# jfjlaros/HUMID

Hardware: AMD Instinct MI355X
Metric: reads/sec deduplicated, 10M PE150 UMI=8 d=1 (higher is better)
Workload: dtype u64; 1 GPU; 10000000 reads/GPU x 1 GPU (one shuffled read set of 10000000 reads, sliced by input order), PE150 UMI=8 in header -> 24-nt packed words (8+8+8), d=1, directional clustering; synthetic molecules=N/4, family 1+Geom(3), p_sub=1e-3, p_N=1e-4; reads_per_gpu=10000000, word_nt=24, distance=1, method=directional

## Files before the change

humid_amd/csrc/humid_exchange.hip:

```cpp
#include "pipeline.hip.h"

extern "C" {

static int compact_nodes_impl(humid_ctx *c, const uint64_t *d_edges, uint64_t n_edges, uint32_t record_stride, u64 id_bound,
                              const uint32_t **d_nodes, uint64_t *n_nodes, const uint64_t **d_compact_edges,
                              const uint32_t **d_node_counts);
static int combo_route_wide(humid_ctx *c, const W2 *d_word, const u32 *d_count, u32 n, u64 id_base, const ComboPlan &plan,
                            u32 combo, u32 n_ranks, const Item3 **d_items, u64 *counts);
static int pairs_keyed_wide(humid_ctx *c, const void *d_items, u32 n, bool interleaved, u64 id_base, const u32 *d_count,
                            const ComboPlan &plan, u32 combo, u32 distance, const u64 **d_records, u64 *n_edges);
static int stage_pairs_share(humid_ctx *c, const u64 *g_word, u32 U, u32 word_nt, u32 distance, u32 part_rank, u32 part_world,
                             u64 *n_edges_out);
namespace {
struct XRange { u64 lo = 1, hi = 0; };

void x_splitters(const std::vector<u64> &hist, u32 P, u32 word_nt, u32 bits, std::vector<XRange> &out) {
  const u32 shift = 2 * word_nt - bits;
  const size_t n_bins = hist.size();
  std::vector<u64> cum(n_bins);
  u64 total = 0;
  for (size_t i = 0; i < n_bins; i++) { total += hist[i]; cum[i] = total; }
  std::vector<size_t> bounds{0};
  for (u32 k = 1; k < P; k++) {
    const u64 target = (total * k + P - 1) / P;
// ... 254 lines not shown
    const void *gw = lw;
    const u32 *gc = lc;
    if (moves && u_total) {
      ENSURE(c->xo_gw, u_total * wb + 16);
      ENSURE(c->xo_gc, u_total * 4 + 16);
      ENSURE(c->s_word, 16);
      ENSURE(c->s_cnt, 16);
      TRY(x_exchange(c, cm, c->s_word.p, ucnt, true, c->xo_gw.p, ucnt, wb));
      TRY(x_exchange(c, cm, c->s_cnt.p, ucnt, true, c->xo_gc.p, ucnt, 4));
      gw = c->xo_gw.p;
      gc = c->xo_gc.as<u32>();
    }
    u64 e_raw = 0;
    if (u_total > 1) {
      if (wide) TRY(edit_edges<W2>(c, (const W2 *)gw, (u32)u_total, n, d, &e_raw, r, P, false));
      else TRY(edit_edges<u64>(c, (const u64 *)gw, (u32)u_total, n, d, &e_raw, r, P, false));
    }
    u64 raw_from[MAX_RANKS], raw_all = 0;
    TRY(x_host_gather(c, cm, &e_raw, 8, raw_from));
    for (u32 q = 0; q < P; q++) raw_all += raw_from[q];
    if (raw_all >= 0x7fffffffull) return fail(c, HUMID_E_OVERFLOW, "too many candidate pairs in the edit-distance search");
    const u64 *all_raw = c->e_raw.as<u64>();
    if (moves && raw_all) {
      ENSURE(c->xo_cross, raw_all * 8 + 16);
      ENSURE(c->e_raw, 16);
      u64 rs[MAX_RANKS];
      for (u32 q = 0; q < P; q++) rs[q] = e_raw;
      TRY(x_exchange(c, cm, c->e_raw.p, rs, true, c->xo_cross.p, raw_from, 8));
      all_raw = c->xo_cross.as<u64>();
    }
    u64 E_e = 0;
    if (raw_all) TRY(unique_edges(c, all_raw, raw_all, (u32)u_total, &E_e));
    XT("edit joins");
    const u32 n_ids = (u32)u_total;
    const u32 nw = (((n_ids + 31) / 32) + 7) & ~7u, nblk = nw / 8;
    c->cg_valid = false;
    c->cg_nblocks = nblk;
    ENSURE(c->cg_bits, (size_t)nw * 4);
    ENSURE(c->cg_nbits, (size_t)nw * 4);
    ENSURE(c->cg_cur, (size_t)(ER_REGIONS * ER_STRIDE + 8) * 4);
    ENSURE(c->xo_cnt, 64 * 4);
    {
      ZeroList z;
      memset(&z, 0, sizeof z);
      z.p[0] = c->cg_bits.as<u32>(); z.n[0] = nw;
      z.p[1] = c->cg_nbits.as<u32>(); z.n[1] = nw;
      z.p[2] = (u32 *)&c->d_ctr[CTR_EDGES]; z.n[2] = 2 * (CTR_GOVER - CTR_EDGES + 1);
      z.p[3] = c->cg_cur.as<u32>(); z.n[3] = ER_REGIONS * ER_STRIDE + 8;
      hipLaunchKernelGGL(k_zero_many, dim3(64), dim3(256), 0, st, z);
    }
    CgStatus cgs;
    u64 M_e = 0;
    if (E_e) {
      hipLaunchKernelGGL(k_mark_pairs, dim3(blocks_for(E_e)), dim3(256), 0, st, (const u64 *)c->e_edges.as<u64>(), (u32)E_e, n_ids,
                         c->cg_bits.as<u32>(), (u32 *)&c->d_ctr[CTR_OVERFULL]);
      CgSource src;
      src.er.e = nullptr; src.er.cap_r = 0; src.er.cur = c->cg_cur.as<u32>(); src.er.far = c->e_edges.as<u64>(); src.er.n_far = (u32)E_e;
      src.recs = nullptr; src.n_recs = 0; src.segs = nullptr; src.cnt_by_id = gc; src.n_ids = n_ids;
      src.pairs_bound = E_e;
      TRY(mark_stage(c, c->ev[EV_GRAPH_BUILT]));
      TRY(cg_build(c, src, method, cgs));
      if (c->h_ctr[CTR_OVERFULL]) return fail(c, HUMID_E_INVALID, "internal: an edit-distance pair outside the unique words");
      M_e = cgs.M;
      TRY(cg_cluster_rest(c, n_ids, cgs.M, cgs.Mbig, method));
    } else {
      ENSURE(c->cg_blk, ((size_t)nblk + 1) * 4);
      ENSURE(c->cg_nblk, ((size_t)nblk + 1) * 4);
      HIPCHK(hipMemsetAsync(c->cg_blk.p, 0, ((size_t)nblk + 1) * 4, st));
      HIPCHK(hipMemsetAsync(c->cg_nblk.p, 0, ((size_t)nblk + 1) * 4, st));
    }
    const GraphArrays cg = cg_arrays(c);
    const BitRank br_in{c->cg_bits.as<u32>(), c->cg_blk.as<u32>()}, br_nc{c->cg_nbits.as<u32>(), c->cg_nblk.as<u32>()};
    const u32 *l_cid = nullptr;
    const u8 *l_ismax = nullptr;
    if (u_local) {
      ENSURE(c->x_lcid, (size_t)u_local * 4);
      ENSURE(c->x_lismax, (size_t)u_local);
      ENSURE(c->xo_ldeg, (size_t)u_local * 4);
      hipLaunchKernelGGL(k_own_results, dim3(blocks_for(u_local)), dim3(256), 0, st, br_in, br_nc, br_nc, (const u32 *)nullptr,
                         (const u32 *)c->cg_nodes.as<u32>(), (const u32 *)cg.cl_of, (const u32 *)cg.maxleaf, (const u32 *)cg.deg, (u32)goff,
                         (u32)u_local, 0u, c->x_lcid.as<u32>(), c->x_lismax.as<u8>(), c->xo_ldeg.as<u32>(),
                         (const u32 *)c->s_first.as<u32>(), (const u32 *)c->s_slot.as<u32>(), c->slot_out.as<u64>(), true);
      c->slots_done = true;
      l_cid = c->x_lcid.as<u32>();
      l_ismax = c->x_lismax.as<u8>();
    }
    HIPCHK(hipGetLastError());
    TRY(read_counters(c, c->cg_nblk.as<u32>() + nblk));
    const u64 clusters_e = u_total - (c->h_ctr[CTR_N - 1] & 0xffffffffull);
    if (clusters_e >= (1ull << 31)) return fail(c, HUMID_E_OVERFLOW, "cluster ids exceed 31 bits");
    XT("graph+ids");
    const u32 *packed = nullptr;
    u64 n_packed = 0;
    TRY(humid_stage_map_dense(c, l_cid, l_ismax, &packed, &n_packed));
    if (n_packed != n_recv) return fail(c, HUMID_E_INVALID, "map_dense returned %llu reads, %llu were counted", (ull)n_packed, (ull)n_recv);
    const u32 *ret = packed;
    if (moves && usable_all) {
      ENSURE(c->xr_ret, n_send * 4 + 8);
      TRY(x_exchange(c, cm, packed, recv_counts, false, c->xr_ret.p, send_counts, 4));
      ret = c->xr_ret.as<u32>();
    }
    if (n_local)
      hipLaunchKernelGGL(k_gather_results, dim3(grid_stride_blocks(n_local)), dim3(256), 0, st, (const u32 *)c->xo_inv.as<u32>(), ret,
                         (u32)n_send, (u32)n_local, d_cluster_id, d_keep);
    HIPCHK(hipGetLastError());
    HIPCHK(hipStreamSynchronize(st));
    XT("return");
    if (xtrace) fprintf(stderr, "[xtrace] rank %u/%u (edit distance) |%s\n", r, P, xt_line.c_str());
    if (summary) {
      memset(summary, 0, sizeof *summary);
      summary->total = total;
      summary->usable = usable;
      summary->unique = u_total;
      summary->clusters = clusters_e;
      summary->edges = E_e;
      summary->nonsingle = M_e;
      summary->ms_total = std::chrono::duration<float, std::milli>(std::chrono::steady_clock::now() - t_begin).count();
    }
    if (info) {
      info->unique_local = u_local;
      info->id_base = goff;
      info->n_nodes = M_e;
      info->n_pairs = E_e;
      info->d_unique_count = lc;
      info->d_unique_degree = u_local ? c->xo_ldeg.as<u32>() : nullptr;
    }
    return HUMID_OK;
  }
  u64 e_mine = 0;
  auto append_pairs = [&](const u64 *rec, u64 n_rec) -> int {
    if (!n_rec) return HUMID_OK;
    HIPCHK(c->xr_eloc.grow_keeping(e_mine * 16, (e_mine + n_rec) * 16, st));
    HIPCHK(hipMemcpyAsync(c->xr_eloc.as<u8>() + e_mine * 16, rec, n_rec * 16, hipMemcpyDeviceToDevice, st));
    e_mine += n_rec;
    return HUMID_OK;
  };
  auto discover_dense = [&]() -> int {
    if (d > 0 && u_total > 1) {
      u32 n_combos = 0, pb2 = 0;
      TRY(humid_stage_plan_info(c, n, d, u_total, &n_combos, &pb2));
      const ComboPlan wplan = make_plan(n, d, u_total, c->force_segments);
      const u64 ibytes = wide ? sizeof(Item3) : 16;
      const u64 *rec = nullptr;
      u64 n_rec = 0;
      if (u_local > 1) {
        if (wide) TRY(pairs_keyed_wide(c, lw, (u32)u_local, false, goff, lc, wplan, 0, d, &rec, &n_rec));
        else TRY(humid_stage_pairs_keyed(c, lw, u_local, 0, goff, lc, n, d, u_total, 0, &rec, &n_rec));
        TRY(append_pairs(rec, n_rec));
      }
      for (u32 cb = 1; cb < n_combos; cb++) {
        const u64 *items = nullptr;
        u64 sc[MAX_RANKS] = {0}, all_sc[MAX_RANKS * MAX_RANKS], rc[MAX_RANKS];
        if (wide) {
          const Item3 *it3 = nullptr;
          TRY(combo_route_wide(c, (const W2 *)lw, lc, (u32)u_local, goff, wplan, cb, P, &it3, sc));
          items = (const u64 *)it3;
        } else
          TRY(humid_stage_combo_route(c, lw, lc, u_local, goff, n, d, u_total, cb, P, &items, sc));
        TRY(x_host_gather(c, cm, sc, P * 8, all_sc));
        u64 n_got = 0;
        for (u32 q = 0; q < P; q++) { rc[q] = all_sc[(size_t)q * P + r]; n_got += rc[q]; }
        if (n_got > 0x7fffffffull) return fail(c, HUMID_E_OVERFLOW, "%llu unique words arrive at rank %u for one combination", (ull)n_got, r);
        u64 items_all = 0;
        for (u32 q = 0; q < P * P; q++) items_all += all_sc[q];
        const u64 *got = items;
        if (moves && items_all) {
// ... 264 lines not shown
  memset(&gs, 0, sizeof gs);
  CgStatus cgs;
  u64 M_mine = 0;
  if (n_recs_all) {
    u32 n_max = 1;
    for (u32 q = 0; q < REC_SEGS; q++) n_max = std::max(n_max, segs.n[q]);
    hipLaunchKernelGGL(k_mark_segs, dim3(std::min<u32>(blocks_for(n_max), 4096), REC_SEGS), dim3(256), 0, st, segs, n_ids,
                       c->cg_bits.as<u32>(), x_bad);
    CgSource src;
    src.er.e = nullptr; src.er.cap_r = 0; src.er.cur = c->cg_cur.as<u32>(); src.er.far = nullptr; src.er.n_far = 0;
    src.recs = nullptr; src.n_recs = 0; src.segs = &segs; src.cnt_by_id = nullptr; src.n_ids = n_ids;
    src.pairs_bound = n_recs_all;
    TRY(mark_stage(c, c->ev[EV_GRAPH_BUILT]));
    TRY(cg_build(c, src, method, cgs));
    if (c->h_ctr[CTR_OVERFULL]) return fail(c, HUMID_E_INVALID, "a pair record with an index outside the unique words");
    M_mine = cgs.M;
    TRY(cg_cluster_rest(c, n_ids, cgs.M, cgs.Mbig, method));
  } else {
    ENSURE(c->cg_blk, ((size_t)nblk + 1) * 4);
    ENSURE(c->cg_nblk, ((size_t)nblk + 1) * 4);
    HIPCHK(hipMemsetAsync(c->cg_blk.p, 0, ((size_t)nblk + 1) * 4, st));
    HIPCHK(hipMemsetAsync(c->cg_nblk.p, 0, ((size_t)nblk + 1) * 4, st));
  }
  const GraphArrays cg = cg_arrays(c);
  const BitRank br_in{c->cg_bits.as<u32>(), c->cg_blk.as<u32>()}, br_nc{c->cg_nbits.as<u32>(), c->cg_nblk.as<u32>()};
  BitRank br_xc{c->xo_xcbits.as<u32>(), c->xo_xcblk.as<u32>()};

  XT("graph");
  u64 C_x = 0;
  if (X_total && M_mine) {
    ENSURE(c->xo_xroot, (size_t)M_mine + 16);
    HIPCHK(hipMemsetAsync(c->xo_xroot.p, 0, (size_t)M_mine, st));
    hipLaunchKernelGGL(k_flag_xroots, dim3(std::min<u32>(blocks_for(X_total), 4096)), dim3(256), 0, st, segs, 1u, n_ids, br_in,
                       (const u32 *)cg.parent, c->xo_xroot.as<u8>(), by_count);
    hipLaunchKernelGGL(k_xcreator_bits, dim3(blocks_for(M_mine)), dim3(256), 0, st, (const u32 *)cg.cl_of, (const u32 *)cg.parent,
                       (const u8 *)c->xo_xroot.as<u8>(), (const u32 *)c->cg_nodes.as<u32>(), (u32)M_mine, c->xo_xcbits.as<u32>());
  }
  if (X_total) {
    TRY(exscan_in<u32>(c, BitsBlockIn{c->xo_xcbits.as<u32>(), nblk}, c->xo_xcblk.as<u32>(), (u64)nblk + 1));
  }
  hipLaunchKernelGGL(k_own_totals, dim3(1), dim3(64), 0, st, br_nc, br_in, (u32)goff, (u32)u_local, dcnt + 56);
  HIPCHK(hipGetLastError());
  TRY(read_counters(c, dcnt + 56, dcnt + 57, X_total ? c->xo_xcblk.as<u32>() + nblk : nullptr));
  u64 tot_mine[4] = {c->h_ctr[CTR_N - 1] & 0xffffffffull, c->h_ctr[CTR_N - 2] & 0xffffffffull,
                     X_total ? (c->h_ctr[CTR_N - 3] & 0xffffffffull) : 0ull, u_local};
  u64 tot_all[4 * MAX_RANKS];
  TRY(x_host_gather(c, cm, tot_mine, sizeof tot_mine, tot_all));
  u64 creators_before = 0, clusters = 0, M = 0;
  C_x = tot_mine[2];
  for (u32 q = 0; q < P; q++) {
    const u64 cr = tot_all[4 * q + 3] - tot_all[4 * q];
    if (q < r) creators_before += cr;
    clusters += cr;
    M += tot_all[4 * q + 1];
    if (tot_all[4 * q + 2] != C_x) return fail(c, HUMID_E_INVALID, "internal: the ranks disagree on the crossing clusters (%llu vs %llu)", (ull)tot_all[4 * q + 2], (ull)C_x);
  }
  if (clusters >= (1ull << 31)) return fail(c, HUMID_E_OVERFLOW, "cluster ids exceed 31 bits");
  const u32 *xcid_all = nullptr;
  if (C_x) {
    ENSURE(c->xo_xcid, C_x * 4 + 16);
    hipLaunchKernelGGL(k_xcreator_ids, dim3(blocks_for(nw)), dim3(256), 0, st, br_xc, nw, (u32)goff, (u32)u_local, (u32)creators_before,
                       br_nc, c->xo_xcid.as<u32>());
    xcid_all = c->xo_xcid.as<u32>();
    if (moves) {
      ENSURE(c->xo_xcall, (size_t)P * C_x * 4 + 16);
      u64 cs[MAX_RANKS];
      for (u32 q = 0; q < P; q++) cs[q] = C_x;
      TRY(x_exchange(c, cm, c->xo_xcid.p, cs, true, c->xo_xcall.p, cs, 4));
      hipLaunchKernelGGL(k_max_rows, dim3(blocks_for(C_x)), dim3(256), 0, st, (const u32 *)c->xo_xcall.as<u32>(), P, (u32)C_x,
                         c->xo_xcid.as<u32>());
    }
  }
  const u32 *l_cid = nullptr;
  const u8 *l_ismax = nullptr;
  if (u_local) {
    ENSURE(c->x_lcid, (size_t)u_local * 4);
    ENSURE(c->x_lismax, (size_t)u_local);
    ENSURE(c->xo_ldeg, (size_t)u_local * 4);
    hipLaunchKernelGGL(k_own_results, dim3(blocks_for(u_local)), dim3(256), 0, st, br_in, br_nc, br_xc, xcid_all,
                       (const u32 *)c->cg_nodes.as<u32>(), (const u32 *)cg.cl_of, (const u32 *)cg.maxleaf, (const u32 *)cg.deg, (u32)goff,
                       (u32)u_local, (u32)creators_before, c->x_lcid.as<u32>(), c->x_lismax.as<u8>(), c->xo_ldeg.as<u32>(),
                       (const u32 *)c->s_first.as<u32>(), (const u32 *)c->s_slot.as<u32>(), c->slot_out.as<u64>());
    c->slots_done = true;
    HIPCHK(hipGetLastError());
    l_cid = c->x_lcid.as<u32>();
    l_ismax = c->x_lismax.as<u8>();
  }

  XT("ids");
  const u32 *packed = nullptr;
  u64 n_packed = 0;
  TRY(humid_stage_map_dense(c, l_cid, l_ismax, &packed, &n_packed));
  if (n_packed != n_recv) return fail(c, HUMID_E_INVALID, "map_dense returned %llu reads, %llu were counted", (ull)n_packed, (ull)n_recv);
  const u32 *ret = packed;
  if (moves && usable_all) {
    ENSURE(c->xr_ret, n_send * 4 + 8);
    TRY(x_exchange(c, cm, packed, recv_counts, false, c->xr_ret.p, send_counts, 4));
    ret = c->xr_ret.as<u32>();
  }
  if (n_local)
    hipLaunchKernelGGL(k_gather_results, dim3(grid_stride_blocks(n_local)), dim3(256), 0, st, (const u32 *)c->xo_inv.as<u32>(), ret,
                       (u32)n_send, (u32)n_local, d_cluster_id, d_keep);
  HIPCHK(hipGetLastError());
  HIPCHK(hipStreamSynchronize(st));
  XT("return");
  if (xtrace)
    fprintf(stderr, "[xtrace] rank %u/%u reads %llu pairs: mine %llu interior %llu crossing %llu flagged %llu (all ranks) graph %llu nodes |%s\n", r, P,
            (ull)n_local, (ull)e_mine, (ull)n_int, (ull)X_total, (ull)K_total, (ull)M_mine, xt_line.c_str());
  if (summary) {
    *summary = gs;
    summary->total = total;
    summary->usable = usable;
    summary->unique = u_total;
    summary->clusters = clusters;
    summary->edges = E;
    summary->nonsingle = M;
    summary->ms_total = std::chrono::duration<float, std::milli>(std::chrono::steady_clock::now() - t_begin).count();
  }
  if (info) {
    info->unique_local = u_local;
    info->id_base = goff;
    info->n_nodes = M;
    info->n_pairs = E;
    info->d_unique_count = lc;
    info->d_unique_degree = u_local ? c->xo_ldeg.as<u32>() : nullptr;
  }
  return HUMID_OK;
}


int humid_at_least_double(humid_ctx *c, uint64_t a, uint64_t b, int *result) {
  if (!c || !result) return fail(c, HUMID_E_INVALID, "null argument");
  HIPCHK(hipSetDevice(c->device));
  ENSURE(c->scratch, 64);
  hipLaunchKernelGGL(k_at_least_double, dim3(1), dim3(1), 0, c->stream, a, b, c->scratch.as<int>());
  HIPCHK(hipGetLastError());
  HIPCHK(hipMemcpyAsync(result, c->scratch.p, sizeof(int), hipMemcpyDeviceToHost, c->stream));
  HIPCHK(hipStreamSynchronize(c->stream));
  return HUMID_OK;
}

static int stage_heads(humid_ctx *c, const u64 *d_words, u32 n, u32 word_nt, const u64 **heads) {
  if ((uintptr_t)d_words & 15) return fail(c, HUMID_E_INVALID, "wide words must be 16-byte aligned on the device");
  ENSURE(c->xr_heads, (size_t)n * 8 + 16);
  hipLaunchKernelGGL(k_wide_head64, dim3(blocks_for(n)), dim3(256), 0, c->stream, (const W2 *)d_words, n, 2 * (word_nt - 32),
                     c->xr_heads.as<u64>(), 0u);
  HIPCHK(hipGetLastError());
  *heads = c->xr_heads.as<u64>();
  return HUMID_OK;
}

int humid_stage_histogram(humid_ctx *c, const uint64_t *d_words, const uint8_t *d_filtered,
                          uint64_t n_reads, uint32_t word_nt, uint32_t bits, uint32_t *d_hist) {
  if (!c) return fail(nullptr, HUMID_E_INVALID, "ctx is null");
  TRY(check_run_args(c, n_reads, word_nt, 0, 64));
  if (bits == 0 || bits > 12 || bits > 2 * word_nt || !d_hist) return fail(c, HUMID_E_INVALID, "bits must be 1..min(12, 2*word_nt)");
  HIPCHK(hipSetDevice(c->device));
  const u32 n_bins = 1u << bits;
  HIPCHK(hipMemsetAsync(d_hist, 0, n_bins * 4, c->stream));
  if (n_reads) {
    const u64 *keys = d_words;
    if (word_nt > 32) TRY(stage_heads(c, d_words, (u32)n_reads, word_nt, &keys));
    hipLaunchKernelGGL(k_top_hist, dim3(512), dim3(1024), n_bins * 4, c->stream, keys, d_filtered,
                       (u32)n_reads, (u64)0, word_nt >= 32 ? (u64)1 : ((u64)1 << (64 - 2 * word_nt)), bits, d_hist);
  }
  HIPCHK(hipGetLastError());
// ... 24 lines not shown
                            const uint64_t *shard_begin, uint32_t n_shards, uint64_t *counts,
                            uint64_t *n_unique, uint64_t *n_usable) {
  if (!c) return fail(nullptr, HUMID_E_INVALID, "ctx is null");
  state_reset(c);
  TRY(check_run_args(c, n_reads, word_nt, 0, 64));
  const bool wide = word_nt > 32;
  if (wide && d_filtered == nullptr)
    return fail(c, HUMID_E_UNSUPPORTED, "two-word words in the stage-by-stage exchange form: use humid_dedup_run_exchange");
  if (!shard_begin || !counts || n_shards == 0 || n_shards > 4096) return fail(c, HUMID_E_INVALID, "bad argument");
  const bool all_owned = d_filtered == nullptr;
  if (n_reads && (!d_words || (!d_filtered && !all_owned))) return fail(c, HUMID_E_INVALID, "null buffer");
  HIPCHK(hipSetDevice(c->device));
  hipStream_t st = c->stream;
  const u32 N = (u32)n_reads;
  for (u32 q = 0; q <= n_shards; q++)
    if (shard_begin[q] > N || (q && shard_begin[q] < shard_begin[q - 1])) return fail(c, HUMID_E_INVALID, "shard_begin must ascend within [0, n_reads]");
  if (shard_begin[0] != 0 || shard_begin[n_shards] != N) return fail(c, HUMID_E_INVALID, "shards must cover [0, n_reads)");
  humid_summary s;
  memset(&s, 0, sizeof s);
  c->N = c->U = c->E = c->M = c->C = c->usable = 0;
  c->word_nt = word_nt;
  for (u32 q = 0; q < n_shards; q++) counts[q] = 0;
  if (n_unique) *n_unique = 0;
  if (n_usable) *n_usable = 0;
  c->timing.dense_map_timed = false;
  auto counted = [&] {
    if (n_unique) *n_unique = c->U;
    if (n_usable) *n_usable = c->usable;
    return state_publish_count(c, true);
  };
  if (N == 0) return counted();
  if (all_owned) {
    for (u32 q = 0; q < n_shards; q++) counts[q] = shard_begin[q + 1] - shard_begin[q];
    c->N = N;
    TRY(stage_count(c, d_words, nullptr, N, word_nt, range_lo, range_hi, 0, s, true));
    HIPCHK(hipStreamSynchronize(st));
    if (c->usable != N) return fail(c, HUMID_E_INVALID, "a read outside [range_lo, range_hi] in an all-owned count");
    return counted();
  }
  ENSURE(c->opos, ((size_t)N + 1) * 4);
  const u64 *range_keys = d_words;
  if (wide) TRY(stage_heads(c, d_words, N, word_nt, &range_keys));
  {
    ComposeIn<OwnedRangeFlagOp, IotaIn> fin{OwnedRangeFlagOp{range_keys, d_filtered, range_lo, range_hi, N}, IotaIn{}};
    TRY(exscan_in<u32>(c, fin, c->opos.as<u32>(), (u64)N + 1));
  }
  std::vector<u32> got(n_shards + 1);
  for (u32 q = 0; q <= n_shards; q++)
    HIPCHK(hipMemcpyAsync(&got[q], c->opos.as<u32>() + shard_begin[q], 4, hipMemcpyDeviceToHost, st));
  HIPCHK(hipStreamSynchronize(st));
  const u32 n_own = got[n_shards];
  for (u32 q = 0; q < n_shards; q++) counts[q] = got[q + 1] - got[q];
  c->N = n_own;
  if (n_own == 0) return counted();
  ENSURE(c->own_words, (size_t)n_own * (wide ? 16 : 8));
  if (wide) {
    hipLaunchKernelGGL(k_gather_owned_w2, dim3(grid_stride_blocks(N)), dim3(256), 0, st, (const W2 *)d_words, range_keys, d_filtered,
                       (const u32 *)c->opos.as<u32>(), range_lo, range_hi, N, c->own_words.as<W2>());
    HIPCHK(hipGetLastError());
    TRY(stage_count_wide(c, c->own_words.as<W2>(), nullptr, n_own, word_nt, s));
    HIPCHK(hipStreamSynchronize(st));
    return counted();
  }
  hipLaunchKernelGGL(k_gather_owned, dim3(grid_stride_blocks(N)), dim3(256), 0, st, d_words, d_filtered,
                     c->opos.as<u32>(), range_lo, range_hi, N, c->own_words.as<u64>());
  HIPCHK(hipGetLastError());
  TRY(stage_count(c, c->own_words.as<u64>(), nullptr, n_own, word_nt, 0ull, ~0ull, 0, s));
  HIPCHK(hipStreamSynchronize(st));
  return counted();
}

int humid_stage_map_dense(humid_ctx *c, const uint32_t *d_local_cluster_id, const uint8_t *d_local_is_max,
                          const uint32_t **d_packed, uint64_t *n_packed) {
  if (!c) return fail(nullptr, HUMID_E_INVALID, "ctx is null");
  if (!state_dense_count(c)) return fail(c, HUMID_E_STATE, "no preceding humid_stage_count_dense");
  if (!d_packed || !n_packed) return fail(c, HUMID_E_INVALID, "bad argument");
  HIPCHK(hipSetDevice(c->device));
  hipStream_t st = c->stream;
  const u32 N = (u32)c->N, U = (u32)c->U;
  *d_packed = nullptr;
  *n_packed = N;
  if (N == 0) return HUMID_OK;
  if (U && (!d_local_cluster_id || !d_local_is_max)) return fail(c, HUMID_E_INVALID, "null buffer");
  if (U > 0 && !c->slots_done)
    hipLaunchKernelGGL(k_slot_results, dim3(blocks_for(U)), dim3(256), 0, st, d_local_cluster_id, d_local_is_max,
                       c->s_first.as<u32>(), c->s_slot.as<u32>(), U, c->slot_out.as<u64>());
  c->slots_done = false;
  ENSURE(c->own_packed, ((size_t)N + 1) * 4);
  TRY(mark_kernel(c, c->kev[KEV_DENSE_MAP_BEGIN]));
  bool tiled = false;
  if (count_in_partition_order(c)) TRY(unpermute_tiled(c, N, true, c->own_packed.as<u32>(), (u8 *)nullptr, KEV_DENSE_MAP_MID, &tiled));
  if (tiled) {
  } else if (count_bucketed(c)) {
    HIPCHK(hipMemsetAsync(c->own_packed.p, 0, (size_t)N * 4, st));
    hipLaunchKernelGGL(k_read_map_bucket, dim3(c->count_left.n_parts), dim3(256), 0, st, c->pk_vals.as<u32>(),
                       c->pslot.as<u32>(), c->slot_out.as<u64>(), c->pbeg.as<u32>(), c->ucount.as<u32>(), N,
                       c->own_packed.as<u32>());
  } else if (count_in_partition_order(c)) {
    HIPCHK(hipMemsetAsync(c->own_packed.p, 0, (size_t)N * 4, st));
    hipLaunchKernelGGL(k_read_map_part, dim3(grid_stride_blocks(N)), dim3(256), 0, st, c->pk_vals.as<u32>(),
                       c->pslot.as<u32>(), c->slot_out.as<u64>(), N, c->own_packed.as<u32>());
  } else
    hipLaunchKernelGGL(k_read_map_packed, dim3(grid_stride_blocks(N)), dim3(256), 0, st, c->slot_of_read.as<u32>(),
                       c->slot_out.as<u64>(), N, c->own_packed.as<u32>());
  TRY(mark_kernel(c, c->kev[KEV_DENSE_MAP_END]));
  c->timing.dense_map_timed = true;
  HIPCHK(hipGetLastError());
  *d_packed = c->own_packed.as<u32>();
  return HUMID_OK;
}

int humid_stage_unique(humid_ctx *c, const uint64_t **d_word, const uint32_t **d_count,
                       const uint32_t **d_first) {
  if (!c) return fail(nullptr, HUMID_E_INVALID, "ctx is null");
  if (d_word) *d_word = c->U ? c->s_word.as<u64>() : nullptr;
  if (d_count) *d_count = c->U ? c->s_cnt.as<u32>() : nullptr;
  if (d_first) *d_first = c->U ? c->s_first.as<u32>() : nullptr;
  return HUMID_OK;
}

int humid_stage_graph(humid_ctx *c, const uint64_t *d_g_word, const uint32_t *d_g_count,
                      uint64_t n_unique, uint32_t word_nt, uint32_t distance, uint32_t method,
                      const uint32_t **d_cluster_id, const uint8_t **d_is_max, humid_summary *summary) {
  if (!c) return fail(nullptr, HUMID_E_INVALID, "ctx is null");
  state_begin_graph(c);
  TRY(check_run_args(c, n_unique, word_nt, method, 64));
  HIPCHK(hipSetDevice(c->device));
  humid_summary s;
  memset(&s, 0, sizeof s);
  s.unique = n_unique;
  c->distance = distance; c->method = method;
  c->gU = 0; c->E = c->M = c->C = 0;
  if (d_cluster_id) *d_cluster_id = nullptr;
  if (d_is_max) *d_is_max = nullptr;
  if (n_unique) {
    if (!d_g_word || !d_g_count) return fail(c, HUMID_E_INVALID, "null buffer");
    u32 nps = 0;
    if (word_nt > 32) {
      if ((uintptr_t)d_g_word & 15) return fail(c, HUMID_E_INVALID, "wide words must be 16-byte aligned on the device");
      TRY(stage_graph<W2>(c, (const W2 *)d_g_word, d_g_count, (u32)n_unique, word_nt, distance, method, s, nps));
    } else
    TRY(stage_graph(c, d_g_word, d_g_count, (u32)n_unique, word_nt, distance, method, s, nps));
    TRY(n_clusters_from_scan(c, (u32)n_unique, &c->C));
    s.clusters = c->C;
    if (d_cluster_id) *d_cluster_id = c->cid.as<u32>();
    if (d_is_max) *d_is_max = c->ismax.as<u8>();
  }
  HIPCHK(hipStreamSynchronize(c->stream));
  if (summary) *summary = s;
  return state_publish(c, CtxState::STAGE_GRAPH);
}

int humid_stage_map(humid_ctx *c, const uint32_t *d_local_cluster_id, const uint8_t *d_local_is_max,
                    uint64_t n_reads, uint32_t *d_cluster_id, uint8_t *d_keep) {
  if (!c) return fail(nullptr, HUMID_E_INVALID, "ctx is null");
  if (n_reads != c->N) return fail(c, HUMID_E_STATE, "n_reads differs from the preceding humid_stage_count");
  if (n_reads && (!d_cluster_id || !d_keep)) return fail(c, HUMID_E_INVALID, "null buffer");
  if (c->U && (!d_local_cluster_id || !d_local_is_max)) return fail(c, HUMID_E_INVALID, "null buffer");
  HIPCHK(hipSetDevice(c->device));
  if (n_reads) TRY(stage_map(c, d_local_cluster_id, d_local_is_max, (u32)n_reads, d_cluster_id, d_keep));
  HIPCHK(hipStreamSynchronize(c->stream));
  return HUMID_OK;
}

int humid_stage_pairs(humid_ctx *c, const uint64_t *d_g_word, uint64_t n_unique, uint32_t word_nt,
                      uint32_t distance, uint32_t part_rank, uint32_t part_world, const uint64_t **d_edges,
                      uint64_t *n_edges) {
  if (!c) return fail(nullptr, HUMID_E_INVALID, "ctx is null");
  if (!d_edges || !n_edges || part_world == 0 || part_rank >= part_world) return fail(c, HUMID_E_INVALID, "bad argument");
  TRY(check_run_args(c, n_unique, word_nt, 0));
// ... 567 lines not shown
  else
    hipLaunchKernelGGL(k_route_scatter<false>, dim3(n_tiles), dim3(1024), 0, st, d_words, d_filtered, n, rg, n_ranks, shift,
                       (const u8 *)d_table, (const u32 *)tile_cnt, c->x_route.as<u64>(), c->perm.as<u32>(), c->xo_inv.as<u32>());
  HIPCHK(hipGetLastError());
  c->route_checked = false;
  c->route_bad = bad;
  *d_routed = c->x_route.as<u64>();
  *d_perm = c->perm.as<u32>();
  return HUMID_OK;
}

int humid_stage_route_check(humid_ctx *c) {
  if (!c) return fail(nullptr, HUMID_E_INVALID, "ctx is null");
  if (c->route_checked || !c->route_bad) return HUMID_OK;
  HIPCHK(hipSetDevice(c->device));
  u32 flag = 0;
  HIPCHK(hipMemcpyAsync(&flag, c->route_bad, 4, hipMemcpyDeviceToHost, c->stream));
  HIPCHK(hipStreamSynchronize(c->stream));
  c->route_checked = true;
  if (flag) return fail(c, HUMID_E_INVALID, "humid_stage_route: send_counts do not match the reads");
  return HUMID_OK;
}

int humid_stage_exchange_ids(humid_ctx *c, const uint32_t *d_nodes, const uint32_t *d_ccid,
                             const uint8_t *d_cismax, uint64_t n_nodes, uint64_t n_clusters, uint64_t id_base,
                             uint64_t u_local, const uint32_t **d_l_cid, const uint8_t **d_l_ismax) {
  if (!c) return fail(nullptr, HUMID_E_INVALID, "ctx is null");
  if (!d_l_cid || !d_l_ismax) return fail(c, HUMID_E_INVALID, "bad argument");
  if (id_base + u_local > 0xffffffffull || n_nodes > 0xfffffffeull || n_clusters > n_nodes)
    return fail(c, HUMID_E_OVERFLOW, "index out of range");
  *d_l_cid = nullptr;
  *d_l_ismax = nullptr;
  if (u_local == 0) return HUMID_OK;
  if (n_nodes && (!d_nodes || !d_ccid || !d_cismax)) return fail(c, HUMID_E_INVALID, "null buffer");
  HIPCHK(hipSetDevice(c->device));
  hipStream_t st = c->stream;
  const u32 M = (u32)n_nodes, Cc = (u32)n_clusters, goff = (u32)id_base, U = (u32)u_local;
  ENSURE(c->x_creator, ((size_t)Cc + 1) * 4);
  ENSURE(c->x_base, ((size_t)Cc + 1) * 4);
  ENSURE(c->x_mark, ((size_t)U * 2 + 4) * 4);
  ENSURE(c->x_scan, ((size_t)U + 1) * 8);
  ENSURE(c->x_lcid, (size_t)U * 4);
  ENSURE(c->x_lismax, (size_t)U);
  u32 *x_mark = c->x_mark.as<u32>(), *x_markcr = x_mark + U, *x_first = x_markcr + U;
  HIPCHK(hipMemsetAsync(x_mark, 0, ((size_t)U * 2 + 2) * 4, st));
  if (M) {
    HIPCHK(hipMemsetAsync(c->x_creator.p, 0xff, ((size_t)Cc + 1) * 4, st));
    hipLaunchKernelGGL(k_xid_creators, dim3(blocks_for(M)), dim3(256), 0, st, d_ccid, M, Cc, c->x_creator.as<u32>());
    if (Cc)
      hipLaunchKernelGGL(k_xid_base, dim3(blocks_for(Cc)), dim3(256), 0, st, d_nodes, c->x_creator.as<u32>(), M, Cc,
                         goff, U, c->x_base.as<u32>(), x_markcr);
    hipLaunchKernelGGL(k_xid_mark, dim3(blocks_for(M)), dim3(256), 0, st, d_nodes, M, goff, U, x_mark);
    hipLaunchKernelGGL(k_xid_first, dim3(1), dim3(64), 0, st, d_nodes, c->x_creator.as<u32>(), M, Cc, goff,
                       x_first);
  }
  {
    ComposeIn<XidFlagOp, IotaIn> fin{XidFlagOp{x_mark, x_markcr, U}, IotaIn{}};
    TRY(exscan_in<u64>(c, fin, c->x_scan.as<u64>(), (u64)U));
  }
  hipLaunchKernelGGL(k_xid_assign, dim3(blocks_for(U)), dim3(256), 0, st, x_mark, c->x_scan.as<u64>(),
                     x_first, d_ccid, d_cismax, c->x_base.as<u32>(), Cc, goff, U, c->x_lcid.as<u32>(),
                     c->x_lismax.as<u8>());
  HIPCHK(hipGetLastError());
  *d_l_cid = c->x_lcid.as<u32>();
  *d_l_ismax = c->x_lismax.as<u8>();
  return HUMID_OK;
}

int humid_stage_owned_results(humid_ctx *c, const uint32_t *d_local_cluster_id, const uint8_t *d_local_is_max,
                              const uint64_t *shard_begin, uint32_t n_shards, const uint32_t **d_packed,
                              uint64_t *counts) {
  if (!c) return fail(nullptr, HUMID_E_INVALID, "ctx is null");
  if (count_in_partition_order(c)) return fail(c, HUMID_E_STATE, "owned results need the global-table count variant (count_mode 1)");
  if (!shard_begin || !counts || !d_packed || n_shards == 0 || n_shards > 4096) return fail(c, HUMID_E_INVALID, "bad argument");
  HIPCHK(hipSetDevice(c->device));
  hipStream_t st = c->stream;
  const u32 N = (u32)c->N, U = (u32)c->U;
  *d_packed = nullptr;
  for (u32 q = 0; q < n_shards; q++) counts[q] = 0;
  if (N == 0) return HUMID_OK;
  for (u32 q = 0; q <= n_shards; q++)
    if (shard_begin[q] > N || (q && shard_begin[q] < shard_begin[q - 1])) return fail(c, HUMID_E_INVALID, "shard_begin must ascend within [0, n_reads]");
  if (U && (!d_local_cluster_id || !d_local_is_max)) return fail(c, HUMID_E_INVALID, "null buffer");
  if (U > 0)
    hipLaunchKernelGGL(k_slot_results, dim3(blocks_for(U)), dim3(256), 0, st, d_local_cluster_id, d_local_is_max,
                       c->s_first.as<u32>(), c->s_slot.as<u32>(), U, c->slot_out.as<u64>());
  ENSURE(c->opos, ((size_t)N + 1) * 4);
  {
    ComposeIn<OwnedFlagOp, IotaIn> fin{OwnedFlagOp{c->slot_of_read.as<u32>(), N}, IotaIn{}};
    TRY(exscan_in<u32>(c, fin, c->opos.as<u32>(), (u64)N + 1));
  }
  std::vector<u32> got(n_shards + 1);
  for (u32 q = 0; q <= n_shards; q++)
    HIPCHK(hipMemcpyAsync(&got[q], c->opos.as<u32>() + shard_begin[q], 4, hipMemcpyDeviceToHost, st));
  u32 total = 0;
  HIPCHK(hipMemcpyAsync(&total, c->opos.as<u32>() + N, 4, hipMemcpyDeviceToHost, st));
  HIPCHK(hipStreamSynchronize(st));
  if (got[0] != 0 || got[n_shards] != total) return fail(c, HUMID_E_INVALID, "owned reads outside the shard table");
  for (u32 q = 0; q < n_shards; q++) counts[q] = got[q + 1] - got[q];
  ENSURE(c->own_packed, ((size_t)total + 1) * 4);
  if (total)
    hipLaunchKernelGGL(k_owned_results, dim3(grid_stride_blocks(N)), dim3(256), 0, st, c->slot_of_read.as<u32>(),
                       c->opos.as<u32>(), c->slot_out.as<u64>(), N, c->own_packed.as<u32>());
  HIPCHK(hipGetLastError());
  HIPCHK(hipStreamSynchronize(st));
  *d_packed = c->own_packed.as<u32>();
  return HUMID_OK;
}

int humid_stage_owner_perm(humid_ctx *c, const uint64_t *d_words, const uint8_t *d_filtered, uint64_t n_reads,
                           const uint64_t *range_lo, const uint64_t *range_hi, uint32_t n_ranks,
                           const uint32_t **d_perm, uint64_t *counts) {
  return humid_stage_owner_perm_wide(c, d_words, d_filtered, n_reads, 32, range_lo, range_hi, n_ranks, d_perm, counts);
}

int humid_stage_owner_perm_wide(humid_ctx *c, const uint64_t *d_words, const uint8_t *d_filtered, uint64_t n_reads,
                                uint32_t word_nt, const uint64_t *range_lo, const uint64_t *range_hi, uint32_t n_ranks,
                                const uint32_t **d_perm, uint64_t *counts) {
  if (!c) return fail(nullptr, HUMID_E_INVALID, "ctx is null");
  if (word_nt == 0 || word_nt > 64) return fail(c, HUMID_E_UNSUPPORTED, "word_nt must be 1 .. 64");
  if (!range_lo || !range_hi || !counts || !d_perm || n_ranks == 0) return fail(c, HUMID_E_INVALID, "bad argument");
  if (n_ranks > MAX_RANKS) return fail(c, HUMID_E_UNSUPPORTED, "more than %d ranks", MAX_RANKS);
  if (n_reads > 0x7fffffffull) return fail(c, HUMID_E_OVERFLOW, "n_reads exceeds 2^31-1");
  HIPCHK(hipSetDevice(c->device));
  hipStream_t st = c->stream;
  const u32 n = (u32)n_reads;
  *d_perm = nullptr;
  for (u32 q = 0; q < n_ranks; q++) counts[q] = 0;
  if (n == 0) return HUMID_OK;
  if (!d_words || !d_filtered) return fail(c, HUMID_E_INVALID, "null buffer");
  OwnerRanges rg;
  for (u32 q = 0; q < MAX_RANKS; q++) { rg.lo[q] = q < n_ranks ? range_lo[q] : 1; rg.hi[q] = q < n_ranks ? range_hi[q] : 0; }
  ENSURE(c->owner, (size_t)n);
  ENSURE(c->owner_sorted, (size_t)n);
  ENSURE(c->perm, (size_t)n * 4);
  const u64 *range_keys = d_words;
  if (word_nt > 32) TRY(stage_heads(c, d_words, n, word_nt, &range_keys));
  hipLaunchKernelGGL(k_owner_of, dim3(blocks_for(n)), dim3(256), 0, st, range_keys, d_filtered, n, rg, n_ranks,
                     c->owner.as<u8>());
  {
    TRY((sort_pairs_in<u8, u32>(c, PtrIn<u8>{c->owner.as<u8>()}, c->owner_sorted.as<u8>(), IotaIn{}, c->perm.as<u32>(), n, 0, 8)));
  }
  ENSURE(c->small, (size_t)(n_ranks + 2) * 4);
  hipLaunchKernelGGL(k_owner_bounds, dim3(1), dim3(64), 0, st, c->owner_sorted.as<u8>(), n, n_ranks,
                     c->small.as<u32>());
  std::vector<u32> b(n_ranks + 2);
  HIPCHK(hipMemcpyAsync(b.data(), c->small.p, (n_ranks + 2) * 4, hipMemcpyDeviceToHost, st));
  HIPCHK(hipGetLastError());
  HIPCHK(hipStreamSynchronize(st));
  for (u32 q = 0; q < n_ranks; q++) counts[q] = b[q + 1] - b[q];
  *d_perm = c->perm.as<u32>();
  return HUMID_OK;
}

int humid_stage_scatter(humid_ctx *c, const uint32_t *d_perm, const uint32_t *d_packed, uint64_t n_recv,
                        uint64_t n_reads, uint32_t *d_cluster_id, uint8_t *d_keep) {
  if (!c) return fail(nullptr, HUMID_E_INVALID, "ctx is null");
  if (n_recv > n_reads) return fail(c, HUMID_E_INVALID, "n_recv > n_reads");
  HIPCHK(hipSetDevice(c->device));
  hipStream_t st = c->stream;
  if (n_reads) {
    if (!d_cluster_id || !d_keep) return fail(c, HUMID_E_INVALID, "null buffer");
    HIPCHK(hipMemsetAsync(d_cluster_id, 0, (size_t)n_reads * 4, st));
    HIPCHK(hipMemsetAsync(d_keep, 0, (size_t)n_reads, st));
  }
  if (n_recv) {
// ... 10 lines not shown
```

humid_amd/csrc/humid_hip.hip:

```cpp
#include "pipeline.hip.h"
#include "passes.hip.h"

static std::string g_err;
extern "C" __attribute__((visibility("hidden"))) void humid_set_global_error(const char *text) { g_err = text ? text : ""; }

extern "C" {

uint32_t humid_abi_version(void) { return HUMID_ABI_VERSION; }

int humid_device_count(void) {
  int n = 0;
  if (hipGetDeviceCount(&n) != hipSuccess) return 0;
  return n;
}

const char *humid_last_error(const humid_ctx *ctx) { return ctx ? ctx->err.c_str() : g_err.c_str(); }

int humid_ctx_create(humid_ctx **out, int device, void *stream) {
  humid_ctx *c = nullptr;
  if (!out) return fail(nullptr, HUMID_E_INVALID, "out is null");
  *out = nullptr;
  int ndev = 0;
  hipError_t e = hipGetDeviceCount(&ndev);
  if (e != hipSuccess || ndev == 0)
// ... 93 lines not shown
  return HUMID_OK;
}

int humid_ctx_set_option(humid_ctx *c, const char *key, int64_t value) {
  if (!c || !key) return fail(c, HUMID_E_INVALID, "null argument");
  if (strcmp(key, "count_mode") == 0) {
    if (value != 0 && value != 1) return fail(c, HUMID_E_INVALID, "count_mode must be 0 (LDS-partitioned) or 1 (global table)");
    c->count_mode = (int)value;
    return HUMID_OK;
  }
  if (strcmp(key, "count_order") == 0) {
    if (value < -1 || value > 1) return fail(c, HUMID_E_INVALID, "count_order must be -1 (auto), 0 or 1");
    c->count_order = (int)value;
    return HUMID_OK;
  }
  if (strcmp(key, "edit_distance") == 0) {
    c->edit = value != 0;
    return HUMID_OK;
  }
  if (strcmp(key, "keyrank_table_log2") == 0) {
    if (value != 0 && (value < 4 || value > 32)) return fail(c, HUMID_E_INVALID, "keyrank_table_log2 must be 0 (automatic) or 4 .. 32");
    c->kr_force_log2 = (u32)value;
    return HUMID_OK;
  }
  if (strcmp(key, "cells_table_log2") == 0) {
    if (value != 0 && (value < 4 || value > 32)) return fail(c, HUMID_E_INVALID, "cells_table_log2 must be 0 (automatic) or 4 .. 32");
    c->cd_force_log2 = (u32)value;
    return HUMID_OK;
  }
  if (strcmp(key, "whitelist_coop") == 0) {
    c->wl_coop = value != 0;
    return HUMID_OK;
  }
  if (strcmp(key, "tile_partition") == 0) {
    c->use_tile_partition = value != 0;
    return HUMID_OK;
  }
  if (strcmp(key, "coop_big") == 0) {
    c->coop_big = value != 0;
    return HUMID_OK;
  }
  if (strcmp(key, "kernel_timing") == 0) {
    c->kev_on = value != 0;
    return HUMID_OK;
  }
  if (strcmp(key, "test_fail_before_gather") == 0) {
    c->x_test_fail_after = (int)value;
    return HUMID_OK;
  }
  if (strcmp(key, "records8") == 0) {
    c->use_rec8 = value != 0;
    return HUMID_OK;
  }
  if (strcmp(key, "compact_graph") == 0) {
    c->use_compact = value != 0;
    return HUMID_OK;
  }
  if (strcmp(key, "group_buckets") == 0) {
    c->group_buckets = value != 0;
    return HUMID_OK;
  }
  if (strcmp(key, "fused_search") == 0) {
    c->fused_search = value != 0;
    return HUMID_OK;
  }
  if (strcmp(key, "pair_split") == 0) {
    c->pair_split = value != 0;
    return HUMID_OK;
  }
  if (strcmp(key, "group_records") == 0) {
    c->group_records = value != 0;
    return HUMID_OK;
  }
  if (strcmp(key, "overlap_waits") == 0) {
    c->overlap_waits = value != 0;
    return HUMID_OK;
  }
  if (strcmp(key, "device_stamps") == 0) {
    c->device_stamps = value != 0;
    return HUMID_OK;
  }
  if (strcmp(key, "static_tiles") == 0) {
    c->static_tiles = value != 0;
    return HUMID_OK;
  }
  if (strcmp(key, "padded_partition") == 0) {
    c->pt_padded = value != 0;
    return HUMID_OK;
  }
  if (strcmp(key, "force_comm") == 0) {
    c->force_comm = value != 0;
    return HUMID_OK;
  }
  if (strcmp(key, "bucket_walk") == 0) {
    if (value < 0 || value > (1 << 24)) return fail(c, HUMID_E_INVALID, "bucket_walk must be 0 (no limit) .. 2^24");
    c->walk_max = (u32)value;
    return HUMID_OK;
  }
  if (strcmp(key, "optical_walk") == 0) {
    if (value < 0 || value > (1 << 24)) return fail(c, HUMID_E_INVALID, "optical_walk must be 0 (no limit) .. 2^24");
    c->op_walk = (u32)value;
    return HUMID_OK;
  }
  if (strcmp(key, "plan_segments") == 0) {
    if (value < 0 || value > 32) return fail(c, HUMID_E_INVALID, "plan_segments must be 0 (auto) .. 32");
    c->force_segments = (u32)value;
    return HUMID_OK;
  }
  if (strcmp(key, "long_key_bits") == 0) {
    if (value < 1 || value > 64) return fail(c, HUMID_E_INVALID, "long_key_bits must be 1 .. 64");
    c->lg_key_bits = (u32)value;
    return HUMID_OK;
  }
  if (strcmp(key, "accum_tile") == 0) {
    if (value < 64 || value > ACC_TILE || (value & (value - 1))) return fail(c, HUMID_E_INVALID, "accum_tile must be a power of two, 64 .. %u", ACC_TILE);
    c->ac_tile = (u32)value;
    return HUMID_OK;
  }
  return fail(c, HUMID_E_INVALID, "unknown option '%s'", key);
}

int humid_dedup_run_device(humid_ctx *c, const uint64_t *d_words, const uint8_t *d_filtered,
                           uint64_t n_reads, uint32_t word_nt, uint32_t distance, uint32_t method,
                           uint32_t *d_cluster_id, uint8_t *d_keep, humid_summary *summary) {
  if (!c) return fail(nullptr, HUMID_E_INVALID, "ctx is null");
  return with_word_type(word_nt, [&](auto *w) {
    return run_device(c, (decltype(w))d_words, d_filtered, n_reads, word_nt, distance, method, d_cluster_id, d_keep, summary);
  });
}

int humid_dedup_run_grouped_device(humid_ctx *c, const uint64_t *d_words, const uint32_t *d_group,
                                   const uint8_t *d_filtered, uint64_t n_reads, uint32_t word_nt, uint32_t n_groups,
                                   uint32_t distance, uint32_t method, uint32_t *d_cluster_id, uint8_t *d_keep,
                                   humid_summary *summary) {
  if (!c) return fail(nullptr, HUMID_E_INVALID, "ctx is null");
  return with_word_type(word_nt, [&](auto *w) {
    return run_grouped_device(c, (decltype(w))d_words, d_group, d_filtered, n_reads, word_nt, n_groups, distance, method,
                              d_cluster_id, d_keep, summary);
  });
}

int humid_dedup_run_keyed_device(humid_ctx *c, const uint64_t *d_words, const uint64_t *d_key, const uint8_t *d_filtered,
                                 uint64_t n_reads, uint32_t word_nt, uint32_t distance, uint32_t method,
                                 uint32_t *d_cluster_id, uint8_t *d_keep, humid_summary *summary) {
  if (!c) return fail(nullptr, HUMID_E_INVALID, "ctx is null");
  return with_word_type(word_nt, [&](auto *w) {
    return run_keyed_device(c, (decltype(w))d_words, d_key, d_filtered, n_reads, word_nt, distance, method, d_cluster_id, d_keep,
                            summary);
  });
}

int humid_dedup_run_keyed_corrected_device(humid_ctx *c, const uint64_t *d_words, const uint64_t *d_key,
                                           const uint8_t *d_filtered, uint64_t n_reads, uint32_t word_nt, uint32_t distance,
                                           uint32_t method, uint32_t *d_cluster_id, uint8_t *d_keep, humid_summary *summary) {
  if (!c) return fail(nullptr, HUMID_E_INVALID, "ctx is null");
  return with_word_type(word_nt, [&](auto *w) {
    return run_keyed_corrected_device(c, (decltype(w))d_words, d_key, d_filtered, n_reads, word_nt, distance, method,
                                      d_cluster_id, d_keep, summary);
  });
}

int humid_dedup_run_keyed_posterior_device(humid_ctx *c, const uint64_t *d_words, const uint64_t *d_key, const uint8_t *d_qual,
                                           const uint8_t *d_filtered, uint64_t n_reads, uint32_t word_nt, uint32_t distance,
                                           uint32_t method, uint32_t min_odds, uint32_t *d_cluster_id, uint8_t *d_keep,
                                           humid_summary *summary) {
  if (!c) return fail(nullptr, HUMID_E_INVALID, "ctx is null");
// ... 1618 lines not shown
```

humid_amd/csrc/kernels_cgraph.hip.h:

```cpp
#ifndef HUMID_KERNELS_CGRAPH_HIP_H
#define HUMID_KERNELS_CGRAPH_HIP_H

#include "common.hip.h"
#include "kernels_graph.hip.h"
#include "kernels_cluster.hip.h"

#define ER_REGIONS 64u
#define ER_STRIDE 32u
struct EdgeRegs {
  u64 *e;
  u32 cap_r;
  u32 *cur;
  const u64 *far;
  u32 n_far;
};
__device__ __forceinline__ u32 er_count(const EdgeRegs &er, u32 r) {
  if (r == ER_REGIONS) return er.n_far;
  const u32 c = er.cur[r * ER_STRIDE];
  return c < er.cap_r ? c : er.cap_r;
}
__device__ __forceinline__ u64 *er_at(const EdgeRegs &er, u32 r, u32 k) {
  return r == ER_REGIONS ? (u64 *)er.far + k : er.e + (size_t)r * er.cap_r + k;
}

// ... 488 lines not shown
          maxleaf[a] = (cb > ca) ? b : a;
          cl_size[a] = ca + cb;
        } else if (at_least_double(cb, ca)) {
          cl_of[a] = a + 1; cl_of[b] = a + 1;
          maxleaf[a] = b;
          cl_size[a] = ca + cb;
        } else if (at_least_double(ca, cb)) {
          cl_of[a] = a + 1; cl_of[b] = a + 1;
          maxleaf[a] = a;
          cl_size[a] = ca + cb;
        } else {
          cl_of[a] = a + 1; maxleaf[a] = a; cl_size[a] = ca;
          cl_of[b] = b + 1; maxleaf[b] = b; cl_size[b] = cb;
        }
      }
    }
    const u64 bm = __ballot(small_root);
    if (bm) {
      u32 base = 0;
      if (lane == 0) base = atomicAdd(&lroots_n, (u32)__popcll(bm));
      base = __shfl(base, 0);
      if (small_root) lroots[base + (u32)__popcll(bm & ((1ull << lane) - 1ull))] = a;
    }
    if ((++round & (CC_ROOTS / 256u - 1u)) == 0) {
      __syncthreads();
      const u32 cntl = lroots_n;
      if (cntl) {
        if (threadIdx.x == 0) lroots_base = (u32)atomicAdd(&ctr[CTR_SMALLROOTS], (ull)cntl);
        __syncthreads();
        for (u32 k = threadIdx.x; k < cntl; k += blockDim.x) small_roots[lroots_base + k] = lroots[k];
        __syncthreads();
        if (threadIdx.x == 0) lroots_n = 0;
      }
      __syncthreads();
    }
  }
  __syncthreads();
  const u32 cntl = lroots_n;
  if (cntl) {
    if (threadIdx.x == 0) lroots_base = (u32)atomicAdd(&ctr[CTR_SMALLROOTS], (ull)cntl);
    __syncthreads();
    for (u32 k = threadIdx.x; k < cntl; k += blockDim.x) small_roots[lroots_base + k] = lroots[k];
  }
  const u32 tb = block_sum(mb, lds);
  if (threadIdx.x == 0 && tb) atomicAdd(&ctr[CTR_MEMBERS], (ull)tb);
}

static __global__ void __launch_bounds__(256)
k_noncreator_bits(const u32 *__restrict__ cl_of, const u32 *__restrict__ nodes, u32 m, u32 *bits, const u32 *__restrict__ m_dev = nullptr) {
  HUMID_GUARD_LAST_VGPR();
  const u32 c = blockIdx.x * blockDim.x + threadIdx.x;
  if (m_dev && *m_dev < m) m = *m_dev;
  if (c >= m || cl_of[c] == c + 1) return;
  const u32 u = nodes[c];
  atomicOr(&bits[u >> 5], 1u << (u & 31));
}

static __global__ void __launch_bounds__(256)
k_finalize_leaves(BitRank in_graph, BitRank noncreator, const u32 *__restrict__ nodes, const u32 *__restrict__ cl_of,
                  const u32 *__restrict__ maxleaf, u32 n, const u32 *__restrict__ s_first, const u32 *__restrict__ s_slot,
                  u64 *__restrict__ slot_out, u32 *__restrict__ cid_out, u8 *__restrict__ ismax_out,
                  const u32 *__restrict__ any_pair = nullptr, const u32 *__restrict__ pair_res = nullptr) {
  HUMID_GUARD_LAST_VGPR();
  const u32 u = blockIdx.x * blockDim.x + threadIdx.x;
  if (u >= n) return;
  u32 g = u;
  bool mx = true;
  if (pair_res && !((any_pair[u >> 5] >> (u & 31)) & 1u)) {
  } else if (br_test(in_graph, u)) {
    const u32 c = br_rank(in_graph, u);
    const u32 cc = cl_of[c] - 1u;
    g = nodes[cc];
    mx = maxleaf[cc] == c;
  } else if (pair_res) {
    const u32 p = pair_res[u];
    g = p & 0x7fffffffu;
    mx = (p >> 31) != 0;
  }
  const u32 id = 1u + g - br_rank(noncreator, g);
  if (slot_out) slot_out[s_slot ? s_slot[u] : u] = ((u64)(mx ? s_first[u] : NONE32) << 32) | id;
  if (cid_out) { cid_out[u] = id; ismax_out[u] = mx ? 1 : 0; }
}

static __global__ void __launch_bounds__(256)
k_expand_leaves(BitRank in_graph, const u32 *__restrict__ nodes, const u32 *__restrict__ cdeg, const u32 *__restrict__ ccl_of,
                const u32 *__restrict__ cmaxleaf, const u64 *__restrict__ ccl_size, const u32 *__restrict__ cnt, u32 n,
                u32 *__restrict__ deg, u32 *__restrict__ cl_of, u32 *__restrict__ maxleaf, u64 *__restrict__ cl_size) {
  HUMID_GUARD_LAST_VGPR();
  const u32 u = blockIdx.x * blockDim.x + threadIdx.x;
  if (u > n) return;
  if (u == n) { deg[u] = 0; return; }
  if (!br_test(in_graph, u)) { deg[u] = 0; cl_of[u] = u + 1; maxleaf[u] = u; cl_size[u] = cnt[u]; return; }
  const u32 c = br_rank(in_graph, u);
  deg[u] = cdeg[c];
  const u32 cc = ccl_of[c] - 1u;
  cl_of[u] = nodes[cc] + 1u;
  if (cc == c) { maxleaf[u] = nodes[cmaxleaf[c]]; cl_size[u] = ccl_size[c]; }
}
static __global__ void __launch_bounds__(256)
k_expand_rows(const u32 *__restrict__ nodes, const u32 *__restrict__ coff, const u32 *__restrict__ cidx, u32 m,
              const u32 *__restrict__ off, u32 *__restrict__ idx) {
  HUMID_GUARD_LAST_VGPR();
  const u32 c = blockIdx.x * blockDim.x + threadIdx.x;
  if (c >= m) return;
  const u32 b = coff[c], d = coff[c + 1] - b, o = off[nodes[c]];
  for (u32 k = 0; k < d; k++) idx[o + k] = nodes[cidx[b + k]];
}

#endif
```

humid_amd/csrc/kernels_part8.hip.h:

```cpp
#ifndef HUMID_KERNELS_PART8_HIP_H
#define HUMID_KERNELS_PART8_HIP_H

#include "common.hip.h"
#include "kernels_count.hip.h"
#include "kernels_part.hip.h"

#define P8_CAP2_LOG 10u
#define P8_CAP2 (1u << P8_CAP2_LOG)
#define P8_RPT (P8_CAP2 / 256u)

struct RecKey {
  u64 lo, scale;
  u32 z, kbits;
  u32 pow2;
  __host__ __device__ __forceinline__ u64 operator()(u64 w) const { return ((w - lo) * scale) >> z; }
  __device__ __forceinline__ u64 word(u64 k) const {
    if (pow2) return lo + k;
    const u64 x = k << z, q = x / scale;
    return lo + q + ((x - q * scale) ? 1u : 0u);
  }
};

struct Reads8 {
  const u64 *words;
// ... 108 lines not shown
    if (blockIdx.x >= tprefix[1u << d1]) return;
    if (threadIdx.x == 0) {
      u32 c, b, n;
      pt_tile_of(tprefix, cbase, 1u << d1, blockIdx.x, cap1, c, b, n);
      s_c = c; s_beg = b; s_cnt = n;
    }
    for (u32 b = threadIdx.x; b < nb; b += PT_THREADS) cnt[b] = 0;
    __syncthreads();
    coarse = s_c; t_beg = s_beg; t_cnt = s_cnt;
  }
  PH(1);
  const u32 fshift = ibits + kbits - d1 - d2;
  u64 rec[PT_IPT];
  u32 binrank[PT_IPT];
#pragma unroll
  for (u32 q = 0; q < PT_IPT; q++) {
    const u32 j = threadIdx.x + q * PT_THREADS;
    binrank[q] = NONE32;
    if (j < t_cnt) rec[q] = in[t_beg + j];
  }
#pragma unroll
  for (u32 q = 0; q < PT_IPT; q++) {
    const u32 j = threadIdx.x + q * PT_THREADS;
    if (j < t_cnt) {
      const u32 bin = (u32)(rec[q] >> fshift) & (nb - 1);
      binrank[q] = bin << 16 | atomicAdd(&cnt[bin], 1u);
    }
  }
  PH(2);
  __syncthreads();
  PH(3);
  block_exscan_512(cnt, loff, nb, wsum);
  PH(4);
  if (threadIdx.x < nb) {
    const u32 c = cnt[threadIdx.x];
    const u32 g = (coarse << d2) | threadIdx.x;
    const u32 had = c ? atomicAdd(&cursor2[g], c) : 0u;
    goff[threadIdx.x] = had;
    room[threadIdx.x] = had >= P8_CAP2 ? 0u : P8_CAP2 - had;
    if (had + c > P8_CAP2) ctr[CTR_SPECIAL] = 1;
  }
  PH(5);
#pragma unroll
  for (u32 q = 0; q < PT_IPT; q++)
    if (binrank[q] != NONE32) srec[loff[binrank[q] >> 16] + (binrank[q] & 0xffffu)] = rec[q];
  __syncthreads();
  PH(6);
  const u64 gbase = (u64)(coarse << d2) << P8_CAP2_LOG;
  p8_write_bins(srec, loff, nb, p8_group(loff[nb], nb), out, [&](u32 bin, u32 k) -> u64 {
    return k < room[bin] ? gbase + ((u64)bin << P8_CAP2_LOG) + goff[bin] + k : ~0ull;
  });
  PH(7);
  PH_END(2, 7, (blockIdx.x & 15u) == 3u);
}

#define DR_SPILL 64u
#define DR_SLOTS (LDS_SLOTS + DR_SPILL)
__device__ __forceinline__ void dr_run_bounds(const u32 *lbits, u32 w, u32 bit, u32 bw, u32 &start, u32 &end) {
  const u32 zb = ~bw & ((1u << bit) - 1u);
  if (zb) start = (w << 5) + (32u - (u32)__clz((int)zb));
  else {
    u32 ww = w;
    start = w << 5;
    while (ww > 0) {
      const u32 pz = ~lbits[ww - 1];
      if (pz) { start = ((ww - 1) << 5) + (32u - (u32)__clz((int)pz)); break; }
      ww--;
      start = ww << 5;
    }
  }
  const u32 za = bit < 31 ? (~bw & ~((2u << bit) - 1u)) : 0u;
  if (za) end = (w << 5) + (u32)__ffs((int)za) - 1u;
  else {
    u32 ww = w + 1;
    while (true) {
      const u32 nz = ~lbits[ww];
      if (nz) { end = (ww << 5) + (u32)__ffs((int)nz) - 1u; break; }
      ww++;
    }
  }
}
#define DR_WORDS (DR_SLOTS / 32u)
#define DR_EARLY 1u
static __global__ void __launch_bounds__(256)
k_dedup_rec(u64 *recs, const u32 *__restrict__ cursor2, u32 n_reads, u32 pb, u32 d1, u32 ibits, RecKey rk,
            u64 *__restrict__ pad_word, uint2 *__restrict__ pad_cf, u64 *__restrict__ agg, ull *ctr, u64 *stamp = nullptr) {
  HUMID_GUARD_LAST_VGPR();
  device_stamp(stamp);
  PH_DECL;
  __shared__ u64 lkey[DR_SLOTS];
  __shared__ uint2 lcf[DR_SLOTS];
  __shared__ unsigned short lslot_of[P8_CAP2];
  __shared__ u32 lbits[DR_WORDS + 2], lpre[DR_WORDS + 2];
  __shared__ u32 lcount;
  const u32 g = blockIdx.x;
  const size_t beg = (size_t)g << P8_CAP2_LOG;
  PH(0);
  u64 rq[P8_RPT];
#pragma unroll
  for (u32 q = 0; q < DR_EARLY; q++) rq[q] = recs[beg + threadIdx.x + 256u * q];
  u32 n = cursor2[g];
  if (n > P8_CAP2) n = P8_CAP2;
  if (n == 0) {
    if (threadIdx.x == 0) agg[g] = 0;
    return;
  }
#pragma unroll
  for (u32 q = DR_EARLY; q < P8_RPT; q++) {
    const u32 i = threadIdx.x + 256u * q;
    if (i < n) rq[q] = recs[beg + i];
  }
  for (u32 s = threadIdx.x; s < DR_SLOTS; s += 256) { lkey[s] = EMPTY_KEY; lcf[s] = make_uint2(0u, NONE32); }
  if (threadIdx.x < DR_WORDS + 2) lbits[threadIdx.x] = 0;
  if (threadIdx.x == 0) lcount = 0;
  __syncthreads();
  PH(1);
  const u32 rbits = rk.kbits - d1, d2 = pb - d1;
  const u64 top = (u64)(g >> d2) << rbits;
  const u64 imask = (1ull << ibits) - 1ull;
  const int hs = (int)rk.kbits - (int)pb - (int)LDS_SLOT_BITS;
  auto home = [&](u64 k) -> u32 { return hs >= 0 ? (u32)(k >> hs) & (LDS_SLOTS - 1) : (u32)k & ((1u << (rk.kbits - pb)) - 1u); };
  bool bad = false;
  u32 sq[P8_RPT];
#pragma unroll
  for (u32 q = 0; q < P8_RPT; q++) {
    const u32 i = threadIdx.x + 256u * q;
    sq[q] = NONE32;
    if (i >= n) continue;
    const u64 k = top | (rq[q] >> ibits);
    const u32 v = (u32)(rq[q] & imask);
    if (v >= n_reads) { bad = true; continue; }
    u32 s = home(k);
    bool claimed = false;
    while (true) {
      u64 cur = lkey[s];
      if (cur == EMPTY_KEY) { cur = atomicCAS((ull *)&lkey[s], EMPTY_KEY, (ull)k); claimed = cur == EMPTY_KEY; }
      if (claimed || cur == k) break;
      if (++s >= DR_SLOTS) break;
    }
    if (s >= DR_SLOTS) { bad = true; continue; }
    sq[q] = s;
    atomicAdd(&lcf[s].x, 1u);
    atomicMin(&lcf[s].y, v);
    if (claimed) {
      lslot_of[atomicAdd(&lcount, 1u)] = (unsigned short)s;
      atomicOr(&lbits[s >> 5], 1u << (s & 31));
    }
  }
  if (bad) ctr[CTR_OVERFULL] = 1;
  PH(2);
  __syncthreads();
  PH(3);
  const u32 n_uniq = lcount;
  const u32 lane = threadIdx.x & 63;
  if ((threadIdx.x & ~63u) < n_uniq) {
    const u32 pc = lane < DR_WORDS ? (u32)__popc(lbits[lane]) : 0u;
    u32 incl = pc;
    incl = wave_incl_scan(incl);
    if (lane < DR_WORDS) lpre[lane] = incl - pc;
  }
  for (u32 li = threadIdx.x; li < n_uniq; li += 256) {
    const u32 sl = lslot_of[li];
    const u32 w = sl >> 5, bit = sl & 31;
    const u32 bw = lbits[w];
    u32 r = lpre[w] + (u32)__popc(bw & ((1u << bit) - 1u));
    const bool left = bit ? ((bw >> (bit - 1)) & 1u) != 0 : (w > 0 && (lbits[w - 1] >> 31) != 0);
    const bool right = bit < 31 ? ((bw >> (bit + 1)) & 1u) != 0 : (lbits[w + 1] & 1u) != 0;
    const u64 k = lkey[sl];
    if (left || right) {
      u32 start, end, smaller = 0;
      dr_run_bounds(lbits, w, bit, bw, start, end);
      if (end > DR_SLOTS) end = DR_SLOTS;
      for (u32 j = start; j < end; j++) smaller += lkey[j] < k ? 1u : 0u;
      r = r - (sl - start) + smaller;
    }
    const uint2 cf = lcf[sl];
    pad_word[beg + r] = rk.word(k);
    pad_cf[beg + r] = cf;
    lcf[sl].y = r;
  }
  if (threadIdx.x == 0) agg[g] = ((u64)n << 32) | n_uniq;
  PH(4);
  __syncthreads();
  PH(5);
#pragma unroll
  for (u32 q = 0; q < P8_RPT; q++) {
    const u32 i = threadIdx.x + 256u * q;
    if (i >= n) continue;
    const u32 li = sq[q] != NONE32 ? lcf[sq[q]].y : NONE32;
    recs[beg + i] = ((u64)(li < n ? (u32)beg + li : NOSLOT) << 32) | (u32)(rq[q] & imask);
  }
  PH(6);
  PH_END(0, 6, (g & 255u) == 77u);
}

static __global__ void __launch_bounds__(256)
k_compact_padded8(const u64 *__restrict__ pad_word, const uint2 *__restrict__ pad_cf, const u64 *__restrict__ agg,
                  const u64 *__restrict__ abase, u32 n_parts, u64 *__restrict__ s_word, u32 *__restrict__ s_slot,
                  u32 *__restrict__ s_cnt, u32 *__restrict__ s_first) {
  HUMID_GUARD_LAST_VGPR();
  const u32 wave = (blockIdx.x * blockDim.x + threadIdx.x) >> 6;
  const u32 lane = threadIdx.x & 63;
  if (wave >= n_parts) return;
  const u32 beg = wave << P8_CAP2_LOG, uc = (u32)agg[wave], ub = (u32)abase[wave];
  for (u32 j = lane; j < uc; j += 64) {
    s_word[ub + j] = pad_word[beg + j];
    s_slot[ub + j] = beg + j;
    const uint2 cf = pad_cf[beg + j];
    s_cnt[ub + j] = cf.x;
    s_first[ub + j] = cf.y;
  }
}

template <u32 NBMAX, u32 UIPT = 8u>
__global__ void __launch_bounds__(1024, NBMAX <= 1536 ? 8 : 4)
k_unperm_bins8(const u64 *__restrict__ recs, const u32 *__restrict__ cursor2, const u64 *__restrict__ slot_out, u32 n_parts,
               u32 B, u32 n_reads, u32 wshift, u32 n_bins, u32 *ucur, u64 *__restrict__ rec) {
  HUMID_GUARD_LAST_VGPR();
  constexpr u32 UTILE = PT_THREADS * UIPT;
  __shared__ u64 srec[UTILE];
  __shared__ u32 cnt[NBMAX], loff[NBMAX + 1], goff[NBMAX], wsum[16];
  __shared__ u32 bpre[65];
  PH_DECL;
  PH(0);
  const u32 g0 = blockIdx.x * B;
  if (g0 >= n_parts) return;
  const u32 nbk = (n_parts - g0 < B) ? n_parts - g0 : B;
  if (threadIdx.x < 64) {
    u32 c = threadIdx.x < nbk ? cursor2[g0 + threadIdx.x] : 0u;
    if (c > P8_CAP2) c = P8_CAP2;
    u32 incl = c;
    incl = wave_incl_scan(incl);
    bpre[threadIdx.x + 1] = incl;
    if (threadIdx.x == 0) bpre[0] = 0;
  }
  __syncthreads();
  const u32 T = bpre[nbk];
  const u64 inv_mean = T ? (((u64)nbk << 32) / T) : 0;
  PH(1);
  for (u32 c0 = 0; c0 < T; c0 += UTILE) {
    for (u32 b = threadIdx.x; b < n_bins; b += PT_THREADS) cnt[b] = 0;
    __syncthreads();
    u64 in[UIPT], r64[UIPT];
    u32 binrank[UIPT];
#pragma unroll
    for (u32 q = 0; q < UIPT; q++) {
      const u32 r = c0 + threadIdx.x + q * PT_THREADS;
      binrank[q] = NONE32;
      if (r < T) {
        u32 lo = (u32)(((u64)r * inv_mean) >> 32);
        if (lo >= nbk) lo = nbk - 1;
        while (bpre[lo] > r) lo--;
        while (bpre[lo + 1] <= r) lo++;
        in[q] = recs[((size_t)(g0 + lo) << P8_CAP2_LOG) + (r - bpre[lo])];
        binrank[q] = 0;
      }
    }
    PH(2);
#pragma unroll
    for (u32 q = 0; q < UIPT; q++) {
      if (binrank[q] == NONE32) continue;
      const u32 r = (u32)in[q], sl = (u32)(in[q] >> 32);
      binrank[q] = NONE32;
      if (r < n_reads && sl != NOSLOT) {
        const u64 o = slot_out[sl];
        const u32 c = (u32)o | (((u32)(o >> 32) == r) ? 0x80000000u : 0u);
        r64[q] = ((u64)c << 32) | r;
        const u32 bin = r >> wshift;
        binrank[q] = bin << 16 | atomicAdd(&cnt[bin], 1u);
      }
    }
    PH(3);
    __syncthreads();
    PH(4);
    {
      const u32 a = 2 * threadIdx.x, b = a + 1;
      const u32 ca = a < n_bins ? cnt[a] : 0u, cb = b < n_bins ? cnt[b] : 0u;
      const u32 s = ca + cb;
      const u32 lane = threadIdx.x & 63, wv = threadIdx.x >> 6;
      u32 incl = s;
      incl = wave_incl_scan(incl);
      if (lane == 63) wsum[wv] = incl;
      __syncthreads();
      u32 before = 0;
      for (u32 k = 0; k < wv; k++) before += wsum[k];
      const u32 ex = before + incl - s;
      if (a < n_bins) loff[a] = ex;
      if (b < n_bins) loff[b] = ex + ca;
      if (threadIdx.x == 1023) loff[n_bins] = before + incl;
    }
    __syncthreads();
    PH(5);
    for (u32 b = threadIdx.x; b < n_bins; b += PT_THREADS) {
      const u32 c = cnt[b];
      goff[b] = (b << wshift) + (c ? atomicAdd(&ucur[b], c) : 0u);
    }
    PH(6);
#pragma unroll
    for (u32 q = 0; q < UIPT; q++)
      if (binrank[q] != NONE32) srec[loff[binrank[q] >> 16] + (binrank[q] & 0xffffu)] = r64[q];
    __syncthreads();
    PH(7);
    p8_write_bins(srec, loff, n_bins, p8_group(loff[n_bins], n_bins), rec,
                  [&](u32 bin, u32 k) -> u64 { return (u64)goff[bin] + k; });
    __syncthreads();
    PH(8);
  }
  PH_END(3, 8, (blockIdx.x & 15u) == 3u);
}

#define PW_TILE 4096u
#define PW_IPT (PW_TILE / PT_THREADS)
#include "kernels_wide.hip.h"

__device__ __forceinline__ u64 pw_key(const W2 &x, u32 hbits, const RecKey &rk) {
  return rk((hbits >= 64 ? x.hi : ((x.hi << (64 - hbits)) | (x.lo >> hbits))) >> WIDE_KEY_DROP);
}

template <class Dst>
__device__ __forceinline__ void pw_write_bins(const W2 *sw, const u32 *si, const u32 *loff, u32 nb, u32 G, W2 *__restrict__ ow,
                                              u32 *__restrict__ oi, Dst dst) {
  const u32 lane = threadIdx.x & 63, wv = threadIdx.x >> 6, n_waves = blockDim.x >> 6;
  const u32 per_wave = 64 / G, sub = lane / G, gl = lane % G;
  for (u32 b0 = wv * per_wave; b0 < nb; b0 += n_waves * per_wave) {
    const u32 bin = b0 + sub;
    if (bin >= nb) continue;
    const u32 beg = loff[bin], n = loff[bin + 1] - beg;
    for (u32 k = gl; k < n; k += G) {
      const u64 d = dst(bin, k);
      if (d != ~0ull) { ow[d] = sw[beg + k]; oi[d] = si[beg + k]; }
    }
  }
}

template <int LEVEL>
__global__ void __launch_bounds__(1024)
k_pw_scatter(const W2 *__restrict__ w_in, const u8 *__restrict__ filtered, const u32 *__restrict__ i_in, u32 n_reads, u32 hbits,
             RecKey rk, const u32 *__restrict__ tprefix, const u32 *__restrict__ cbase, u32 d1, u32 d2, u32 cap1, u32 *cursor,
             W2 *__restrict__ w_out, u32 *__restrict__ i_out, ull *ctr) {
  HUMID_GUARD_LAST_VGPR();
  __shared__ W2 sw[PW_TILE];
  __shared__ u32 si[PW_TILE];
  __shared__ u32 cnt[PT_MAXBINS], loff[PT_MAXBINS + 1], goff[PT_MAXBINS], room[PT_MAXBINS], wsum[8];
  __shared__ u32 s_c, s_beg, s_cnt;
  const u32 nb = 1u << (LEVEL == 1 ? d1 : d2);
  u32 t_beg, t_cnt, coarse = 0;
  if (LEVEL == 1) {
    t_beg = blockIdx.x * PT_TILE;
    t_cnt = (t_beg >= n_reads) ? 0u : ((n_reads - t_beg < PT_TILE) ? n_reads - t_beg : PT_TILE);
// ... 197 lines not shown
```

humid_amd/csrc/pass_timing.hip.h:

```cpp
#pragma once

#define EVREC(ev, st) do { c->timing_left.event_records++; HIPCHK(hipEventRecord((ev), (st))); } while (0)

enum PairPhase : u32 { PAIRS_FILL = KEV_PAIRS_FILL, PAIRS_COUNT = KEV_PAIRS_COUNT };
static inline KernelEvent kev_pairs(PairPhase phase, u32 combo, u32 end) { return (KernelEvent)(phase + 2 * combo + end); }

static inline bool kernel_marks_on(const humid_ctx *c) { return c->kev_on && !c->timing.kernels_quiet; }
static int mark_stage(humid_ctx *c, hipEvent_t e) {
  if (!c->timing.lean) EVREC(e, c->stream);
  return HUMID_OK;
}
static int mark_kernel(humid_ctx *c, hipEvent_t e) {
  if (kernel_marks_on(c)) EVREC(e, c->stream);
  return HUMID_OK;
}
static int mark_frame(humid_ctx *c, hipEvent_t e) {
  if (!c->timing.stamp_timed) EVREC(e, c->stream);
  return HUMID_OK;
}
static int mark_pairs(humid_ctx *c, PairPhase phase, u32 combo, u32 end) {
  return combo < KEV_PAIR_COMBOS ? mark_kernel(c, c->kev[kev_pairs(phase, combo, end)]) : HUMID_OK;
}

struct PassTimingGuard {
  PassTiming &t;
  PassTimingGuard(humid_ctx *c, bool offer_stamps) : t(c->timing) {
    t.lean = !c->kev_on && getenv("HUMID_ALL_EVENTS") == nullptr;
    t.stamp_live = t.stamp_timed = false;
    t.stamp_ok = offer_stamps;
  }
  ~PassTimingGuard() { t.lean = t.stamp_ok = t.stamp_live = t.stamp_timed = false; }
  PassTimingGuard(const PassTimingGuard &) = delete;
};

static inline void pass_begin(humid_ctx *c, u64 n_reads, u32 word_nt) {
  c->timing.unperm_tiled = false;
  c->N = n_reads; c->U = c->E = c->M = c->C = c->usable = 0;
  c->word_nt = word_nt;
  c->gU = 0;
}
static inline void pass_begin(humid_ctx *c, u64 n_reads, u32 word_nt, u32 distance, u32 method) {
  pass_begin(c, n_reads, word_nt);
  c->distance = distance; c->method = method;
}

static int gkey_check(humid_ctx *c);
static int timing_tail(humid_ctx *c, humid_summary &s, u32 n_pair_segs, bool per_kernel = true) {
  const PassTiming &t = c->timing;
  TimingLeft &left = c->timing_left;
  const bool timed = t.stamp_timed;
  const bool delivered = t.stamp_live && !c->no_poll;
  if (delivered) {
    for (u32 k = 0; k < STAMP_N; k++) left.stamps[k] = c->h_ctr[STAMP_AT + k];
    left.stamp_live = true;
    left.stamp_timed = timed;
  }
  if (!timed) HIPCHK(hipEventSynchronize(c->ev[EV_PASS_END]));
  if (!t.lean) {
    HIPCHK(hipEventElapsedTime(&s.ms_count, c->ev[EV_PASS_START], c->ev[EV_COUNT_END]));
    HIPCHK(hipEventElapsedTime(&s.ms_neighbours, c->ev[EV_COUNT_END], c->ev[EV_GRAPH_BUILT]));
    HIPCHK(hipEventElapsedTime(&s.ms_cluster, c->ev[EV_GRAPH_BUILT], c->ev[EV_CLUSTERS_DONE]));
    HIPCHK(hipEventElapsedTime(&s.ms_map, c->ev[EV_CLUSTERS_DONE], c->ev[EV_PASS_END]));
  }
  if (timed && delivered) {
    s.ms_total = (float)((double)(left.stamps[STAMP_END] - left.stamps[STAMP_START]) / 1e5);
    s.ms_k_insert = (float)((double)(left.stamps[STAMP_K1] - left.stamps[STAMP_K0]) / 1e5);
  } else if (!timed) HIPCHK(hipEventElapsedTime(&s.ms_total, c->ev[EV_PASS_START], c->ev[EV_PASS_END]));
  TRY(gkey_check(c));
  if (!timed) HIPCHK(hipEventElapsedTime(&s.ms_k_insert, c->kev[KEV_INSERT_BEGIN], c->kev[KEV_INSERT_END]));
  const bool kernels = per_kernel && c->kev_on;
  if (kernels && count_in_partition_order(c))
    HIPCHK(hipEventElapsedTime(&s.ms_k_map, c->ev[EV_CLUSTERS_DONE], c->kev[KEV_MAP_MID]));
  else s.ms_k_map = s.ms_map;
  if (!kernels) return HUMID_OK;
  if (count_in_partition_order(c) && t.unperm_tiled) HIPCHK(hipEventElapsedTime(&s.ms_k_unperm, c->kev[KEV_MAP_MID], c->kev[KEV_UNPERM_END]));
  if (count_part_timed(c)) HIPCHK(hipEventElapsedTime(&s.ms_k_part, c->kev[KEV_PART_BEGIN], c->kev[KEV_PART_END]));
  HIPCHK(hipEventElapsedTime(&s.ms_k_cluster, c->kev[KEV_CLUSTER_BEGIN], c->kev[KEV_CLUSTER_END]));
  for (u32 g = 0; g < n_pair_segs; g++) {
    float ms = 0;
    HIPCHK(hipEventElapsedTime(&ms, c->kev[kev_pairs(PAIRS_COUNT, g, 0)], c->kev[kev_pairs(PAIRS_COUNT, g, 1)]));
    s.ms_k_pairs += ms;
    if (c->E > 0 && !c->cg_valid) {
      HIPCHK(hipEventElapsedTime(&ms, c->kev[kev_pairs(PAIRS_FILL, g, 0)], c->kev[kev_pairs(PAIRS_FILL, g, 1)]));
      s.ms_k_pairs += ms;
    }
  }
  return HUMID_OK;
}
```

humid_amd/csrc/pipeline.hip.h:

```cpp
#ifndef HUMID_PIPELINE_HIP_H
#define HUMID_PIPELINE_HIP_H

#include <fcntl.h>
#include <sys/mman.h>
#include <sys/stat.h>
#include <unistd.h>

#include <atomic>
#include <cerrno>
#include <chrono>
#include <type_traits>
#include <utility>

#include "common.hip.h"
#include "prims.hip.h"
#include "kernels_count.hip.h"
#include "kernels_part.hip.h"
#include "kernels_part8.hip.h"
#include "kernels_graph.hip.h"
#include "kernels_cluster.hip.h"
#include "kernels_cgraph.hip.h"
#include "kernels_map.hip.h"
#include "kernels_xchg.hip.h"
#include "kernels_wide.hip.h"
// ... 2 lines not shown
#include "kernels_gstats.hip.h"
#include "kernels_whitelist.hip.h"
#include "kernels_wlpost.hip.h"
#include "kernels_segments.hip.h"
#include "kernels_cells.hip.h"
#include "kernels_paired.hip.h"
#include "kernels_accum.hip.h"
#include "kernels_long.hip.h"

struct Arena {
  char *base = nullptr;
  size_t size = 0, used = 0;
  void *take(size_t bytes) {
    const size_t at = (used + 255) & ~(size_t)255;
    if (!base || at + bytes > size) return nullptr;
    used = at + bytes;
    return base + at;
  }
};

struct DBuf {
  void *p = nullptr;
  size_t cap = 0;
  bool in_arena = false;
  DBuf() = default;
  DBuf(const DBuf &) = delete;
  DBuf &operator=(const DBuf &) = delete;
  DBuf(DBuf &&o) noexcept { *this = std::move(o); }
  DBuf &operator=(DBuf &&o) noexcept {
    if (this != &o) { release(); p = o.p; cap = o.cap; in_arena = o.in_arena; o.p = nullptr; o.cap = 0; o.in_arena = false; }
    return *this;
  }
  ~DBuf() { release(); }
  hipError_t ensure(size_t bytes, Arena *arena = nullptr) {
    if (bytes <= cap) return hipSuccess;
    release();
    size_t want = bytes + bytes / 8 + 256;
    if (arena) {
      if (void *q = arena->take(bytes + 256)) { p = q; cap = bytes + 256; in_arena = true; return hipSuccess; }
    }
    hipError_t e = hipMalloc(&p, want);
    if (e != hipSuccess) { p = nullptr; return e; }
    cap = want;
    return hipSuccess;
  }
  hipError_t grow_keeping(size_t keep_bytes, size_t need_bytes, hipStream_t stream) {
    if (need_bytes <= cap) return hipSuccess;
    DBuf bigger;
    hipError_t e = bigger.ensure(need_bytes * 2);
    if (e == hipSuccess && keep_bytes) e = hipMemcpyAsync(bigger.p, p, keep_bytes, hipMemcpyDeviceToDevice, stream);
    if (e == hipSuccess) e = hipStreamSynchronize(stream);
    if (e == hipSuccess) *this = std::move(bigger);
    return e;
  }
  void release() { if (p && !in_arena) (void)hipFree(p); p = nullptr; cap = 0; in_arena = false; }
  template <class T> T *as() const { return (T *)p; }
};
static_assert(!std::is_copy_constructible<DBuf>::value && !std::is_copy_assignable<DBuf>::value, "DBuf is move-only");
static_assert(std::is_nothrow_move_constructible<DBuf>::value && std::is_nothrow_move_assignable<DBuf>::value, "DBuf is move-only");

enum RunKind : u8 { RUN_PLAIN, RUN_GROUPED, RUN_KEYED, RUN_CORRECTED };
enum : u32 { CC_NONE = 0, CC_ON, CC_INVALID };
struct CtxState {
  enum Holds : u8 { NOTHING, COUNT, STAGE_GRAPH, HAND_GRAPH, RUN } holds = NOTHING;
  RunKind kind = RUN_PLAIN;
  bool dense = false;
  bool stats_current = false;
  bool paired = false;
  bool long_words = false;
};

enum CountRoad : u8 {
  COUNT_GLOBAL,
  COUNT_LDS_HASHED,
  COUNT_LDS_ORDERED,
  COUNT_REC,
  COUNT_SORTED
};
struct CountLeft {
  CountRoad road = COUNT_GLOBAL;
  u32 n_parts = 0;
  bool part_tiled = false;
  const u32 *cursor2 = nullptr;
};
struct OrderedMemo {
  bool valid = false, fits = false;
  u32 n = 0, nt = 0;
  u64 lo = 0, scale = 0;
};

#define STAMP_N 4
enum StageEvent : u32 {
  EV_PASS_START, EV_COUNT_END, EV_GRAPH_BUILT, EV_CLUSTERS_DONE, EV_PASS_END,
  EV_HOST_FRAME,
  EV_N
};
enum { KEV_PAIR_COMBOS = 8 };
enum KernelEvent : u32 {
  KEV_INSERT_BEGIN, KEV_INSERT_END,
  KEV_CLUSTER_BEGIN, KEV_CLUSTER_END,
  KEV_PAIRS_FILL,
  KEV_PAIRS_COUNT = KEV_PAIRS_FILL + 2 * KEV_PAIR_COMBOS,
  KEV_MAP_MID = KEV_PAIRS_COUNT + 2 * KEV_PAIR_COMBOS,
  KEV_DENSE_MAP_BEGIN, KEV_DENSE_MAP_END,
  KEV_PART_BEGIN, KEV_PART_END,
  KEV_UNPERM_END,
  KEV_DENSE_MAP_MID,
  KEV_N
};
static_assert(EV_N == 6 && KEV_PAIRS_COUNT == 20 && KEV_MAP_MID == 36 && KEV_N == 43, "the event slots");
struct PassTiming {
  bool lean = false;
  bool stamp_ok = false;
  bool stamp_live = false;
  bool stamp_timed = false;
  bool kernels_quiet = false;
  bool unperm_tiled = false;
  bool dense_map_timed = false;
};
struct TimingLeft {
  u64 stamps[STAMP_N] = {};
  bool stamp_live = false, stamp_timed = false;
  u32 event_records = 0;
};

struct humid_ctx {
  int device = 0;
  CtxState state;
  humid_run_roads roads = {};
  RunKind pass_kind = RUN_PLAIN;
  Arena arena;
  hipStream_t stream = nullptr;
  bool own_stream = false;
  std::string err;
  ull *d_ctr = nullptr;
  PsChain *ps_chain = nullptr;
  u32 ps_epoch = 0;
  ull *h_ctr = nullptr;
  ull *h_ctr_dev = nullptr;
  ull ctr_seq = 0;
  u64 *d_stamp = nullptr;
  bool device_stamps = true;
  PassTiming timing;
  TimingLeft timing_left;
  const u32 *gf_valid = nullptr;
  u32 *ucur_clean = nullptr;
  DBuf gf_cur;
  bool gf_padded = true;
  bool no_chain = false;
  bool no_poll = false;
  DBuf in_words, in_filt, in_bases, out_cid, out_keep;
  DBuf stage_in[9], stage_out[3];
  DBuf table, slot_out, slot_of_read, uniq_slot;
  DBuf pk_keys, pk_vals, pbeg, ucount, pusable, ubase, pad_word, pad_cf, pslot;
  DBuf opos, own_packed, owner, owner_sorted, perm, small;
  DBuf pc, poff, share_edges;
  DBuf own_words;
  DBuf heads;
  DBuf small_roots;
  DBuf big_runs;
  DBuf had;
  DBuf e_kx, e_vx, e_ky, e_vy, e_raw, e_sorted, e_edges, e_head, e_hpos;
  DBuf e_runlo, e_nch, e_choff, e_pc2, e_poff2;
  bool edit = false;
  DBuf xr_heads, xr_send, xr_zero;
  DBuf xr_hist, xr_recv, xr_eloc, xr_got, xr_eall, xr_ret;
  DBuf x_slot, x_slot_s, x_cnt, x_cnts, x_rec, x_ncnt, x_route, x_creator, x_base, x_mark, x_markcr, x_scan, x_lcid, x_lismax,
       x_items, x_w, x_id, x_ids, x_ends, x_ends_s, x_head, x_hpos, x_nodes, x_cedges;
  DBuf w_sorted, w_head, w_hpos, w_start, w_heads;
  DBuf cg_edges, cg_cur, cg_far, cg_bits, cg_nbits, cg_blk, cg_nblk, cg_nodes, cg_ncnt, cg_deg, cg_off, cg_idx, cg_parent, cg_csize,
       cg_curs, cg_cl_of, cg_maxleaf, cg_cl_size;
  u64 cg_ecap = 0;
  bool use_compact = true;
  bool cg_valid = false;
  bool cg_expanded = false;
  u32 cg_M = 0, cg_nblocks = 0;
  DBuf cg_multi, cg_rbits, cg_rest, cg_pres;
  bool pair_split = true;
  bool cg_split = false;
  bool cg_full = false;
  bool cg_broken = false;
  bool cg_m_late = false;
  u64 cg_iso = 0, cg_R = 0;
  EdgeRegs cg_er = {};
  u64 cg_pairs_bound = 0;
  u32 cg_method = 0;
  const u32 *ctr_x[3] = {nullptr, nullptr, nullptr};
  DBuf xo_gw, xo_gc;
  DBuf xo_regs, xo_inv;
  u64 xr_ecap = 0;
  DBuf xo_send, xo_int, xo_cross, xo_sel, xo_selall, xo_parent, xo_flag, xo_xroot, xo_xcbits, xo_xcblk, xo_xcid, xo_xcall, xo_ldeg, xo_cnt;
  DBuf pw_a, pw_ai, pw_b, pw_bi;
  DBuf p8_a, p8_b, p8_cur, p8_status;
  bool use_rec8 = true;
  CountLeft count_left;
  DBuf pt_work, unperm_rec, route_tiles;
  bool group_buckets = true;
  bool fused_search = true;
  bool group_records = true;
  u32 gr_rides = 0, gr_orders = 0;
  bool overlap_waits = true;
  bool static_tiles = true;
  u32 wo_waits = 0, wo_overlapped = 0;
  bool pt_padded = true;
  bool use_tile_partition = true;
  int x_test_fail_after = -1, x_gathers = 0;
  bool x_hist_done = false, x_peer_failed = false;
  bool route_checked = true;
  const u32 *route_bad = nullptr;
  OrderedMemo ordered_memo;
  u32 g_wpr = 1;
  bool slots_done = false;
  int count_mode = 0;
  u32 force_segments = 0;
  bool force_comm = false;
  u32 walk_max = PT2_TILE;
  bool coop_big = true;
  int count_order = -1;
  u32 gk_nt = 0;
  u32 gk_epoch = 0;
  u32 gk_word_nt = 0, gk_leaf_nt = 0;
  DBuf gk_words, gk_group_in, gk_bad;
  u32 kr_n = 0;
  u32 kr_cap_log2 = 0;
  u32 kr_force_log2 = 0;
  u32 kr_last_log2 = 0, kr_redo = 0;
  DBuf kr_table, kr_raw, kr_rawslot, kr_keys, kr_slot, kr_key_in;
  DBuf wl_table;
  u64 wl_n = 0;
  u32 wl_nt = 0, wl_log2 = 0;
  bool wl_coop = true;
  u64 bc_N = 0;
  DBuf bc_key, bc_filt, bc_status, bc_counts;
  DBuf wc_counts;
  DBuf bc_qual_in;
  DBuf wp_cnt, wp_slot;
  bool wp_valid = false;
  bool bc_posterior = false;
  SegPlan sg = {};
  u64 sg_distinct[SEG_MAX] = {};
  DBuf sg_table;
  DBuf sg_sum;
  bool sg_sum_valid = false;
  u32 cd_cap_log2 = 0;
  u32 cd_force_log2 = 0;
  DBuf cd_table, cd_cnt, cd_ctr, cd_k0, cd_c0, cd_kkey, cd_kccnt, cd_flag, cd_pos, cd_skey, cd_scnt, cd_tmp;
  DBuf cd_cells, cd_cellcnt, cd_hist_n, cd_hist_first;
  bool cd_valid = false;
  u64 cd_n_cells = 0, cd_n_hist = 0, cd_G = 0;
  u32 cc_state = CC_NONE;
  u32 cc_nt = 0, cc_log2 = 0, cc_grown = 0;
  u64 cc_chunks = 0, cc_reads = 0, cc_usable = 0, cc_invalid = 0, cc_distinct = 0;
  DBuf cc_table, cc_cnt, cc_ctr, cc_pend;
  u32 pr_state = CC_NONE;
  bool wp_prior = false;
  DBuf pr_cnt, pr_ctr;
  u32 gk_groups = 1;
  u32 gs_G = 0;
  DBuf gs_reads, gs_loff, gs_coff, gs_edges, gs_ps;
  DBuf bs_rep, bs_best, bs_ctr;
  DBuf cs_rep, cs_cnt, cs_moff, cs_cur, cs_mem, cs_ctr, cs_big, cs_piece, cs_tab;
  DBuf cs_ooff, cs_ob, cs_oq, cs_depth, cs_errors;
  bool cs_valid = false;
  humid_consensus_summary cs_sum = {};
  bool cs_duplex = false;
  DBuf ds_top, ds_same, ds_other, ds_disagree;
  humid_duplex_summary ds_sum = {};
  DBuf op_rep, op_bctr, op_ctr, op_k0, op_v0, op_v1, op_ct, op_xy, op_vote, op_parent, op_root, op_best, op_gsize;
  u32 op_walk = 64;
  bool pd_run = false;
  DBuf pd_words, pd_strand, pd_mir, pd_top, pd_bottom, pd_ctr;
  u64 pd_N = 0;
  humid_strand_summary pd_sum = {};
  u32 lg_key_bits = 64;
  humid_long_info_t lg_info = {};
  DBuf lg_cand;
  bool ac_on = false;
  bool ac_finished = false;
  u32 ac_nt = 0, ac_cur = 0;
  u32 ac_tile = ACC_TILE;
  u64 ac_U = 0, ac_chunks = 0, ac_total = 0, ac_usable = 0;
  DBuf ac_word[2], ac_cnt[2], ac_first[2];
  DBuf ac_split, ac_tcnt, ac_toff, ac_flag;
  DBuf ac_cid, ac_ismax, ac_lcid, ac_lismax;
  bool ac_keyed = false;
  u32 ac_key_nt = 0, ac_ent_nt = 0;
  u64 ac_G = 0;
  DBuf ac_head, ac_hpos, ac_keys, ac_iword;
  DBuf uniq_word, s_word, s_slot, s_cnt, s_first;
  DBuf deg, nbr_off, nbr_idx, seg_k0, seg_v0, seg_ks, seg_vs, seg_ws, csize, cur;
  DBuf parent, mk0, mk1, cl_of, maxleaf, cl_size, flag, pos, cid, ismax, stk, tmp, scratch;
  hipEvent_t ev[EV_N] = {};
  bool kev_on = false;
  hipEvent_t kev[KEV_N] = {};
  const void *g_word = nullptr;
  const u32 *g_cnt = nullptr;
  u32 gU = 0;
  u32 cap_log2 = 0;
  u64 N = 0, U = 0, E = 0, M = 0, C = 0, usable = 0;
  u32 word_nt = 0, distance = 0, method = 0;
};

extern "C" void humid_set_global_error(const char *text);

static int fail(humid_ctx *c, int code, const char *fmt, ...) {
  char buf[512];
  va_list ap;
  va_start(ap, fmt);
  vsnprintf(buf, sizeof buf, fmt, ap);
  va_end(ap);
  if (c) c->err = buf; else humid_set_global_error(buf);
  return code;
}

#define HIPCHK(expr)                                                                        \
  do {                                                                                      \
    hipError_t _e = (expr);                                                                 \
    if (_e != hipSuccess)                                                                   \
      return fail(c, _e == hipErrorOutOfMemory ? HUMID_E_NOMEM : HUMID_E_HIP, "%s: %s (%s:%d)", \
                  #expr, hipGetErrorString(_e), __FILE__, __LINE__);                        \
  } while (0)

#define STAMP_AT (CTR_N + 2)
static inline bool count_in_partition_order(const humid_ctx *c) { return c->count_left.road != COUNT_GLOBAL; }
static inline bool count_bucketed(const humid_ctx *c) { return c->count_left.n_parts != 0; }
static inline bool count_on_records(const humid_ctx *c) { return c->count_left.road == COUNT_REC; }
static inline bool count_part_timed(const humid_ctx *c) { return c->count_left.part_tiled; }
static inline u32 count_mode_used(const humid_ctx *c) {
  static const u32 mode[] = {1u, 0u, 2u, 2u | 0x100u, 3u};
  return mode[c->count_left.road];
}

enum { STAMP_START = 0, STAMP_K0, STAMP_K1, STAMP_END };

#define ENSURE(buf, bytes) HIPCHK((buf).ensure((bytes), &c->arena))
#define PASS_ENSURE(buf, bytes) HIPCHK((buf).ensure((bytes)))
#define D2H(dst, src, bytes)    \
  do { if ((dst) && (bytes)) HIPCHK(hipMemcpyAsync((dst), (src), (bytes), hipMemcpyDeviceToHost, c->stream)); } while (0)
#define STAGE_OUT(d, j, bytes) do { PASS_ENSURE(c->stage_out[j], (bytes) + 16); (d) = (decltype(d))c->stage_out[j].p; } while (0)
#define STAGE_IN(d, i, h, bytes)                                                              \
  do {                                                                                        \
    PASS_ENSURE(c->stage_in[i], (bytes) + 16);                                                \
    (d) = (decltype(d))c->stage_in[i].p;                                                      \
    if (bytes) HIPCHK(hipMemcpyAsync((d), (h), (bytes), hipMemcpyHostToDevice, c->stream));   \
  } while (0)

static inline u32 blocks_for(u64 n, u32 bs = 256) { return (u32)((n + bs - 1) / bs); }
static inline u32 grid_stride_blocks(u64 n, u32 bs = 256) {
  u64 b = (n + bs - 1) / bs;
  if (b > 256 * 8) b = 256 * 8;
  if (b == 0) b = 1;
  return (u32)b;
}
static inline u32 bits_for(u64 n) {
  u32 b = 0;
  while (b < 64 && ((u64)1 << b) < n) b++;
  return b ? b : 1;
}

template <class K, class V, class KIn, class VIn>
static int sort_pairs_in(humid_ctx *c, KIn kin, K *kout, VIn vin, V *vout, u64 n, u32 b0, u32 b1) {
  if (n == 0) return HUMID_OK;
  if (n > 0xffffffffull) return fail(c, HUMID_E_OVERFLOW, "sort of more than 2^32-1 items");
  ENSURE(c->tmp, (rs_temp_bytes<K, V, true>(n)));
  HIPCHK((rs_sort<K, V, true>(c->tmp.p, kin, kout, vin, vout, n, b0, b1, c->stream)));
  return HUMID_OK;
}
template <class K, class V>
static int sort_pairs(humid_ctx *c, const K *kin, K *kout, const V *vin, V *vout, u64 n, u32 b0, u32 b1) {
  return sort_pairs_in<K, V>(c, PtrIn<K>{kin}, kout, PtrIn<V>{vin}, vout, n, b0, b1);
}
template <class K>
static int sort_keys(humid_ctx *c, const K *kin, K *kout, u64 n, u32 b0, u32 b1) {
  if (n == 0) return HUMID_OK;
  if (n > 0xffffffffull) return fail(c, HUMID_E_OVERFLOW, "sort of more than 2^32-1 items");
  ENSURE(c->tmp, (rs_temp_bytes<K, u32, false>(n)));
  HIPCHK((rs_sort<K, u32, false>(c->tmp.p, PtrIn<K>{kin}, kout, IotaIn{}, (u32 *)nullptr, n, b0, b1, c->stream)));
  return HUMID_OK;
}
template <class T, class In>
static int exscan_in(humid_ctx *c, In in, T *out, u64 n, u64 *stamp = nullptr) {
  ENSURE(c->tmp, ps_scan_scratch_items(n) * sizeof(T) + 256);
  HIPCHK((ps_exscan<T>(in, out, n, (T *)c->tmp.p, c->stream, c->no_chain ? nullptr : c->ps_chain, &c->ps_epoch, stamp)));
  return HUMID_OK;
}
static int exscan_u32(humid_ctx *c, const u32 *in, u32 *out, u64 n) { return exscan_in<u32>(c, PtrIn<u32>{in}, out, n); }

static __global__ void k_publish_counters(const ull *__restrict__ ctr, const u32 *__restrict__ extra32, const u32 *__restrict__ extra32b,
                                   volatile ull *host, ull seq, const u32 *__restrict__ extra32c = nullptr, u64 *stamp = nullptr) {
  HUMID_GUARD_LAST_VGPR();
  if (stamp && threadIdx.x == 0) {
    const u64 t = wall_clock64();
    stamp[STAMP_END] = t;
    host[STAMP_AT + STAMP_START] = stamp[STAMP_START];
    host[STAMP_AT + STAMP_K0] = stamp[STAMP_K0];
    host[STAMP_AT + STAMP_K1] = stamp[STAMP_K1];
    host[STAMP_AT + STAMP_END] = t;
  }
  if (threadIdx.x < CTR_N) {
    ull v = ctr[threadIdx.x];
    if (threadIdx.x == CTR_N - 1 && extra32) v = (v & ~0xffffffffull) | (ull)*extra32;
    if (threadIdx.x == CTR_N - 2 && extra32b) v = (ull)*extra32b;
    if (threadIdx.x == CTR_N - 3 && extra32c) v = (ull)*extra32c;
    host[threadIdx.x] = v;
  }
  __threadfence_system();
  __syncthreads();
  if (threadIdx.x == 0) { host[CTR_N] = seq; __threadfence_system(); }
}
static int read_counters_begin(humid_ctx *c, const u32 *extra32 = nullptr, const u32 *extra32b = nullptr, const u32 *extra32c = nullptr,
// ... 608 lines not shown
                       (u32 *)nullptr, (u32 *)nullptr, c->d_ctr, join_cnt);
    comp_stats(c, U);
  }
  u64 big_mask = 0;
  std::vector<BigRun> h_runs[MAX_COMBOS];
  const BigRun *d_runs[MAX_COMBOS] = {nullptr};
  auto sink = [&](u32 seg) {
    return CsrSink{c->deg.as<u32>(), c->parent.as<u32>(), c->nbr_off.as<u32>(), c->cur.as<u32>(), c->nbr_idx.as<u32>(),
                   c->had.as<u32>() + (size_t)seg * U, join_cnt};
  };
  auto search_pass = [&](int mode) -> int {
    const PairPhase phase = mode == PM_COUNT ? PAIRS_COUNT : PAIRS_FILL;
    for (u32 seg = 0; seg < plan.ncombo; seg++) {
      if (seg && mode == PM_COUNT) TRY(bucket_order<WT>(c, plan, seg, g_word, U, seg_ws<WT>(c, seg, U), seg_vs(c, seg, U)));
      const Walked<WT> w = walked_seg<WT>(c, plan, seg, g_word, U);
      TRY(mark_pairs(c, phase, seg, 0));
      pairs_csr<WT>(c, ps, w, mode, 0u, U, sink(seg), &c->d_ctr[CTR_BIGMASK]);
      if (mode == PM_FILL && (big_mask >> seg & 1)) tiles_csr<WT>(c, ps, w, d_runs[seg], h_runs[seg], PM_FILL, sink(seg));
      TRY(mark_pairs(c, phase, seg, 1));
    }
    HIPCHK(hipGetLastError());
    return HUMID_OK;
  };
  if (search) {
    n_pair_segs = plan.ncombo < 8 ? plan.ncombo : 8;
    ENSURE(c->had, (size_t)plan.ncombo * U * 4);
    TRY(ensure_seg_scratch<WT>(c, plan.ncombo, U));
    TRY(search_pass(PM_COUNT));
    comp_stats(c, U);
  }
  TRY(exscan_u32(c, c->deg.as<u32>(), c->nbr_off.as<u32>(), (u64)U + 1));
  if (search || (given && n_ext_edges)) {
    HIPCHK(hipGetLastError());
    TRY(read_counters(c, c->nbr_off.as<u32>() + U));
    if (c->h_ctr[CTR_OVERFULL]) return fail(c, HUMID_E_INVALID, "malformed edge list (node index out of range)");
    if (c->h_ctr[CTR_EDGES] > 0xffffffffull)
      return fail(c, HUMID_E_OVERFLOW, "%llu neighbour pairs exceed the 32-bit adjacency offsets", (ull)(c->h_ctr[CTR_EDGES] / 2));
    big_mask = search ? c->h_ctr[CTR_BIGMASK] : 0;
    u64 twoE = c->h_ctr[CTR_N - 1] & 0xffffffffull;
    if (big_mask) {
      road_taken(c, HUMID_ROAD_CSR_TILES);
      for (u32 seg = 0; seg < plan.ncombo; seg++)
        if (big_mask >> seg & 1) {
          const Walked<WT> w = walked_seg<WT>(c, plan, seg, g_word, U);
          TRY(find_big_runs<WT>(c, w.W, U, w.mask, ps.walk_max, seg, h_runs[seg], &d_runs[seg]));
          tiles_csr<WT>(c, ps, w, d_runs[seg], h_runs[seg], PM_COUNT, sink(seg));
          HIPCHK(hipGetLastError());
        }
      HIPCHK(hipMemsetAsync(&c->d_ctr[CTR_EDGES], 0, 3 * sizeof(ull), st));
      HIPCHK(hipMemsetAsync(&c->d_ctr[CTR_SMALLROOTS], 0, sizeof(ull), st));
      HIPCHK(hipMemsetAsync(c->csize.p, 0, (size_t)U * 4, st));
      comp_stats(c, U);
      TRY(scan_total(c, c->deg.as<u32>(), c->nbr_off.as<u32>(), U, &twoE));
      if (c->h_ctr[CTR_EDGES] > 0xffffffffull)
        return fail(c, HUMID_E_OVERFLOW, "%llu neighbour pairs exceed the 32-bit adjacency offsets", (ull)(c->h_ctr[CTR_EDGES] / 2));
    }
    E = twoE / 2;
    M = c->h_ctr[CTR_NONSINGLE];
    Mbig = c->h_ctr[CTR_MEMBERS];
  }
  s.edges = c->E = E;
  s.nonsingle = c->M = M;
  ENSURE(c->nbr_idx, (size_t)(2 * E + 1) * 4);
  if (E > 0) {
    if (given)
      hipLaunchKernelGGL(k_edges_apply<true>, dim3(grid_stride_blocks(n_ext_edges)), dim3(256), 0, st, ext_edges,
                         n_ext_edges, U, (u32 *)nullptr, (u32 *)nullptr, c->nbr_off.as<u32>(),
                         c->cur.as<u32>(), c->nbr_idx.as<u32>(), c->d_ctr);
    else
      TRY(search_pass(PM_FILL));
    hipLaunchKernelGGL(k_sort_lists, dim3(blocks_for(U)), dim3(256), 0, st, c->nbr_off.as<u32>(), U,
                       c->nbr_idx.as<u32>());
  }
  TRY(mark_stage(c, c->ev[EV_GRAPH_BUILT]));

  TRY(cluster_stage(c, g_cnt, U, M, Mbig, method));
  const bool own = ((const void *)g_word == c->s_word.p) && U == (u32)c->U && !given;
  hipLaunchKernelGGL(k_finalize_nodes, dim3(blocks_for(U)), dim3(256), 0, st, c->cl_of.as<u32>(),
                     c->pos.as<u32>(), c->maxleaf.as<u32>(), U, c->cid.as<u32>(), c->ismax.as<u8>(),
                     own ? c->s_first.as<u32>() : (const u32 *)nullptr,
                     own ? c->s_slot.as<u32>() : (const u32 *)nullptr,
                     own ? c->slot_out.as<u64>() : (u64 *)nullptr);
  c->slots_done = own;
  HIPCHK(hipGetLastError());
  n_pair_segs_out = n_pair_segs;
  return HUMID_OK;
}


struct CgSource {
  EdgeRegs er;
  const ulonglong2 *recs;
  u32 n_recs;
  const RecSegs *segs = nullptr;
  const u32 *cnt_by_id;
  u32 n_ids;
  u64 pairs_bound;
  u32 *bits = nullptr;
  bool no_wait = false;
};
struct CgStatus {
  bool overflow = false;
  bool group_over = false;
  u64 wanted = 0, big_mask = 0, E = 0, M = 0, Mbig = 0;
};
static GraphArrays cg_arrays(humid_ctx *c) {
  return GraphArrays{c->cg_deg.as<u32>(), c->cg_parent.as<u32>(), c->cg_csize.as<u32>(), c->cg_off.as<u32>(), c->cg_idx.as<u32>(),
                     c->cg_cl_of.as<u32>(), c->cg_maxleaf.as<u32>(), c->cg_cl_size.as<u64>()};
}
static int cg_build_front(humid_ctx *c, const u32 *bits, u32 n_ids, const u32 *cnt_by_id, u64 nodes_bound) {
  hipStream_t st = c->stream;
  const u32 n_words = (((n_ids + 31) / 32) + 7) & ~7u, n_blk = n_words / 8;
  const size_t Mb = (size_t)std::min<u64>(n_ids, nodes_bound);
  ENSURE(c->cg_blk, ((size_t)n_blk + 1) * 4);
  ENSURE(c->cg_nodes, (Mb + 1) * 4);
  ENSURE(c->cg_ncnt, (Mb + 1) * 4);
  ENSURE(c->cg_deg, (Mb + 2) * 4);
  ENSURE(c->cg_parent, (Mb + 1) * 4);
  ENSURE(c->cg_csize, (Mb + 1) * 4);
  ENSURE(c->cg_curs, (Mb + 1) * 4);
  TRY(exscan_in<u32>(c, BitsBlockIn{bits, n_blk}, c->cg_blk.as<u32>(), (u64)n_blk + 1));
  const BitRank br{bits, c->cg_blk.as<u32>()};
  const GraphArrays g = cg_arrays(c);
  hipLaunchKernelGGL(k_nodes_init, dim3(blocks_for(n_words)), dim3(256), 0, st, br, n_words, cnt_by_id, c->cg_nodes.as<u32>(),
                     c->cg_ncnt.as<u32>(), g.deg, g.parent, g.csize, c->cg_curs.as<u32>(), n_blk);
  HIPCHK(hipGetLastError());
  return HUMID_OK;
}
static int cg_build_back(humid_ctx *c, CgSource &src, u32 method, CgStatus &out) {
  hipStream_t st = c->stream;
  u32 *bits = src.bits ? src.bits : c->cg_bits.as<u32>();
  const u32 n_words = (((src.n_ids + 31) / 32) + 7) & ~7u, n_blk = n_words / 8;
  const u64 pb = std::max<u64>(src.pairs_bound, 1);
  if (2 * pb + 2 > 0xffffffffull) return fail(c, HUMID_E_OVERFLOW, "too many neighbour pairs");
  const u32 Mb = (u32)std::min<u64>(src.n_ids, 2 * pb);
  ENSURE(c->cg_off, ((size_t)Mb + 2) * 4);
  ENSURE(c->cg_idx, (size_t)(2 * pb + 1) * 4);
  ENSURE(c->cg_cl_of, ((size_t)Mb + 1) * 4);
  ENSURE(c->cg_maxleaf, ((size_t)Mb + 1) * 4);
  ENSURE(c->cg_cl_size, ((size_t)Mb + 1) * 8);
  ENSURE(c->small_roots, ((size_t)Mb / 3 + 2) * 4);
  ENSURE(c->small, 64);
  const BitRank br{bits, c->cg_blk.as<u32>()};
  const u32 *m_dev = c->cg_blk.as<u32>() + n_blk;
  const GraphArrays g = cg_arrays(c);
  const u32 r_first = src.er.e ? 0u : ER_REGIONS;
  const bool by_count = (method & 1) == 0;
  if (src.segs) {
    const u32 n_all = src.segs->first[REC_SEGS];
    u32 n_max = 1;
    for (u32 q = 0; q < REC_SEGS; q++) n_max = std::max(n_max, src.segs->n[q]);
    ENSURE(c->cg_far, ((size_t)n_all + 1) * 8);
    hipLaunchKernelGGL(k_segs_relabel, dim3(std::min<u32>(blocks_for(n_max), 4096), REC_SEGS), dim3(256), 0, st, *src.segs, src.n_ids, br,
                       c->cg_far.as<u64>(), c->cg_ncnt.as<u32>(), g.deg, g.parent, by_count);
    src.er.far = c->cg_far.as<u64>();
    src.er.n_far = n_all;
  } else if (src.recs) {
    ENSURE(c->cg_far, ((size_t)src.n_recs + 1) * 8);
    if (src.n_recs)
      hipLaunchKernelGGL(k_records_relabel, dim3(blocks_for(src.n_recs)), dim3(256), 0, st, src.recs, src.n_recs, src.n_ids, br,
                         c->cg_far.as<u64>(), c->cg_ncnt.as<u32>(), g.deg, g.parent, by_count);
    src.er.far = c->cg_far.as<u64>();
    src.er.n_far = src.n_recs;
  } else {
    const u32 gx = (u32)std::min<u64>(std::max<u64>(blocks_for(std::max<u64>(src.er.cap_r, src.er.n_far)), 1), 4096);
    hipLaunchKernelGGL(k_pairs_relabel, dim3(gx, ER_REGIONS + 1 - r_first), dim3(256), 0, st, src.er, br, (const u32 *)c->cg_ncnt.as<u32>(),
// ... 206 lines not shown
      continue;
    }
    if (given) {
      u32 h_bad = 0;
      HIPCHK(hipMemcpyAsync(&h_bad, bad, 4, hipMemcpyDeviceToHost, st));
      HIPCHK(hipStreamSynchronize(st));
      if (h_bad) return fail(c, HUMID_E_INVALID, "malformed edge list (node index out of range)");
    }
    if (search && cgs.big_mask && !far) {
      const u64 big_mask = cgs.big_mask;
      u64 got = 0;
      for (int phase = 0; phase < 2; phase++) {
        u64 at = 0;
        for (u32 seg = 0; seg < nseg; seg++) {
          if (!(big_mask >> seg & 1)) continue;
          if (seg && !ordered_seg[seg]) {
            TRY(bucket_order<WT>(c, plan, seg, g_word, U, seg_ws<WT>(c, seg, U), seg_vs(c, seg, U), true));
            ordered_seg[seg] = true;
            c->gr_orders++;
          }
          const Walked<WT> w = walked_seg<WT>(c, plan, seg, g_word, U);
          std::vector<BigRun> runs;
          const BigRun *d_runs = nullptr;
          TRY(find_big_runs<WT>(c, w.W, U, w.mask, ps.walk_max, seg, runs, &d_runs));
          if (!runs.back().tile0) continue;
          const ull start = phase ? at : 0;
          HIPCHK(hipMemcpyAsync(&c->d_ctr[CTR_SPECIAL], &start, sizeof(ull), hipMemcpyHostToDevice, st));
          HIPCHK(hipStreamSynchronize(st));
          tiles_emit<WT>(c, ps, w, d_runs, runs, phase ? PM_EMIT_FILL : PM_EMIT_COUNT,
                         EmitSink{nullptr, nullptr, c->cg_far.as<u64>(), &c->d_ctr[CTR_SPECIAL]});
          HIPCHK(hipGetLastError());
          TRY(read_counters(c));
          if (phase == 0) got += c->h_ctr[CTR_SPECIAL]; else at = c->h_ctr[CTR_SPECIAL];
        }
        if (phase == 0) {
          if (got > 0x7fffffffull) return fail(c, HUMID_E_OVERFLOW, "%llu neighbour pairs exceed the 32-bit adjacency offsets", (ull)got);
          ENSURE(c->cg_far, (size_t)(got + 1) * 8);
        }
      }
      far = c->cg_far.as<u64>();
      n_far = got;
      if (n_far) { road_taken(c, HUMID_ROAD_FAR_TILES); continue; }
    }
    if (split) {
      c->cg_er = er;
      c->cg_pairs_bound = ecap + n_far;
    } else { E = cgs.E; M = cgs.M; Mbig = cgs.Mbig; }
    if (search && 2 * (cgs.wanted + cgs.wanted / 4 + ER_REGIONS * 64) < c->cg_ecap) c->cg_ecap = cgs.wanted + cgs.wanted / 4 + ER_REGIONS * 64;
    break;
  }
  const u32 *late_m = nullptr;
  bool fetch = false;
  if (split) {
    c->cg_split = true;
    c->cg_method = method;
    c->cg_iso = n_iso; c->cg_R = R;
    E = n_iso + R;
    if (R > 0) {
      CgSource src;
      src.er.e = nullptr; src.er.cap_r = 0; src.er.cur = c->cg_cur.as<u32>(); src.er.far = c->cg_rest.as<u64>(); src.er.n_far = (u32)R;
      src.recs = nullptr; src.n_recs = 0; src.cnt_by_id = g_cnt; src.n_ids = U;
      src.pairs_bound = R;
      src.bits = c->cg_rbits.as<u32>();
      src.no_wait = true;
      if (c->overlap_waits) TRY(cg_build_back(c, src, method, cgs));
      else TRY(cg_build(c, src, method, cgs));
      late_m = c->cg_blk.as<u32>() + n_blk;
      fetch = R >= SMALL_COMP;
      c->cg_m_late = !fetch;
      M = std::min<u64>(U, 2 * R);
      Mbig = 0;
    } else TRY(mark_kernel(c, c->kev[KEV_CLUSTER_BEGIN]));
  }
  s.edges = c->E = E;
  TRY(mark_stage(c, c->ev[EV_GRAPH_BUILT]));
  u64 M_rest = 0;
  TRY(cg_cluster_rest(c, U, M, Mbig, method, late_m, fetch, &M_rest));
  if (split) M = 2 * n_iso + (fetch ? M_rest : 0);
  s.nonsingle = c->M = M;
  c->cg_M = split ? 0u : (u32)M;
  const GraphArrays g = cg_arrays(c);
  const bool own = ((const void *)g_word == c->s_word.p) && U == (u32)c->U;
  if (!own) { ENSURE(c->cid, (size_t)U * 4); ENSURE(c->ismax, (size_t)U); }
  hipLaunchKernelGGL(k_finalize_leaves, dim3(blocks_for(U)), dim3(256), 0, st,
                     BitRank{split ? c->cg_rbits.as<u32>() : c->cg_bits.as<u32>(), c->cg_blk.as<u32>()},
                     BitRank{c->cg_nbits.as<u32>(), c->cg_nblk.as<u32>()}, c->cg_nodes.as<u32>(), (const u32 *)g.cl_of,
                     (const u32 *)g.maxleaf, U, own ? c->s_first.as<u32>() : (const u32 *)nullptr,
                     own ? c->s_slot.as<u32>() : (const u32 *)nullptr, own ? c->slot_out.as<u64>() : (u64 *)nullptr,
                     own ? (u32 *)nullptr : c->cid.as<u32>(), own ? (u8 *)nullptr : c->ismax.as<u8>(),
                     split ? (const u32 *)c->cg_bits.as<u32>() : (const u32 *)nullptr,
                     split ? (const u32 *)c->cg_pres.as<u32>() : (const u32 *)nullptr);
  c->slots_done = own;
  c->cg_valid = true;
  HIPCHK(hipGetLastError());
  n_pair_segs_out = nseg < 8 ? nseg : 8;
  return HUMID_OK;
}

static int n_clusters_compact(humid_ctx *c, u32 U, u64 *out) {
  TRY(read_counters(c, c->cg_nblk.as<u32>() + c->cg_nblocks, c->cg_m_late ? c->cg_blk.as<u32>() + c->cg_nblocks : (const u32 *)nullptr,
                    nullptr, c->timing.stamp_live ? c->d_stamp : nullptr));
  *out = (u64)U - (c->h_ctr[CTR_N - 1] & 0xffffffffull);
  if (c->cg_m_late) { c->M += c->h_ctr[CTR_N - 2] & 0xffffffffull; c->cg_m_late = false; }
  return HUMID_OK;
}

static int cg_build_full(humid_ctx *c) {
  hipStream_t st = c->stream;
  struct Quiet { PassTiming &t; ~Quiet() { t.kernels_quiet = false; } } quiet{c->timing};
  c->timing.kernels_quiet = true;
  struct RunsWaits { humid_ctx *c; u32 w, o; ~RunsWaits() { c->wo_waits = w; c->wo_overlapped = o; } } waits{c, c->wo_waits, c->wo_overlapped};
  {
    ZeroList z;
    memset(&z, 0, sizeof z);
    z.p[0] = (u32 *)&c->d_ctr[CTR_EDGES]; z.n[0] = 2 * (CTR_GOVER - CTR_EDGES + 1);
    hipLaunchKernelGGL(k_zero_many, dim3(1), dim3(256), 0, st, z);
  }
  CgSource src;
  src.er = c->cg_er; src.recs = nullptr; src.n_recs = 0; src.cnt_by_id = c->g_cnt; src.n_ids = c->gU;
  src.pairs_bound = c->cg_pairs_bound;
  CgStatus cgs;
  TRY(cg_build(c, src, c->cg_method, cgs));
  if (cgs.E != c->E) return fail(c, HUMID_E_INVALID, "internal: the full graph has %llu pairs, the run found %llu", (ull)cgs.E, (ull)c->E);
  if (cgs.M > 0) TRY(cluster_kernels(c, cg_arrays(c), c->cg_ncnt.as<u32>(), (u32)cgs.M, cgs.M, cgs.Mbig, c->cg_method, true));
  HIPCHK(hipStreamSynchronize(st));
  c->cg_M = (u32)cgs.M;
  c->cg_full = true;
  return HUMID_OK;
}
static int cg_ensure_full(humid_ctx *c) {
  if (!c->cg_valid || !c->cg_split || c->cg_full) return HUMID_OK;
  if (c->cg_broken) return fail(c, HUMID_E_STATE, "the graph of this run could not be built when it was first asked for; run again");
  const int rc = cg_build_full(c);
  if (rc != HUMID_OK) c->cg_broken = true;
  return rc;
}

static int expand_compact(humid_ctx *c) {
  if (!c->cg_valid || c->cg_expanded) return HUMID_OK;
  TRY(cg_ensure_full(c));
  hipStream_t st = c->stream;
  const u32 U = c->gU, M = c->cg_M;
  const u64 E = c->E;
  if (U == 0) { c->cg_expanded = true; return HUMID_OK; }
  ENSURE(c->deg, ((size_t)U + 1) * 4);
  ENSURE(c->nbr_off, ((size_t)U + 1) * 4);
  ENSURE(c->nbr_idx, (size_t)(2 * E + 1) * 4);
  ENSURE(c->cl_of, (size_t)U * 4);
  ENSURE(c->maxleaf, (size_t)U * 4);
  ENSURE(c->cl_size, (size_t)U * 8);
  ENSURE(c->flag, (size_t)U * 4);
  ENSURE(c->pos, ((size_t)U + 1) * 4);
  ENSURE(c->cid, (size_t)U * 4);
  ENSURE(c->ismax, (size_t)U);
  const BitRank br{c->cg_bits.as<u32>(), c->cg_blk.as<u32>()};
  hipLaunchKernelGGL(k_expand_leaves, dim3(blocks_for((u64)U + 1)), dim3(256), 0, st, br, c->cg_nodes.as<u32>(), c->cg_deg.as<u32>(),
                     c->cg_cl_of.as<u32>(), c->cg_maxleaf.as<u32>(), c->cg_cl_size.as<u64>(), c->g_cnt, U, c->deg.as<u32>(),
                     c->cl_of.as<u32>(), c->maxleaf.as<u32>(), c->cl_size.as<u64>());
  TRY(exscan_u32(c, c->deg.as<u32>(), c->nbr_off.as<u32>(), (u64)U + 1));
  if (M)
    hipLaunchKernelGGL(k_expand_rows, dim3(blocks_for(M)), dim3(256), 0, st, c->cg_nodes.as<u32>(), c->cg_off.as<u32>(),
                       c->cg_idx.as<u32>(), M, c->nbr_off.as<u32>(), c->nbr_idx.as<u32>());
  hipLaunchKernelGGL(k_creator_flags, dim3(blocks_for(U)), dim3(256), 0, st, c->cl_of.as<u32>(), U, c->flag.as<u32>());
  TRY(exscan_u32(c, c->flag.as<u32>(), c->pos.as<u32>(), U));
  hipLaunchKernelGGL(k_finalize_nodes, dim3(blocks_for(U)), dim3(256), 0, st, c->cl_of.as<u32>(), c->pos.as<u32>(),
                     c->maxleaf.as<u32>(), U, c->cid.as<u32>(), c->ismax.as<u8>(), (const u32 *)nullptr, (const u32 *)nullptr,
                     (u64 *)nullptr);
  HIPCHK(hipGetLastError());
  HIPCHK(hipStreamSynchronize(st));
  c->cg_expanded = true;
  return HUMID_OK;
}

static int unique_edges(humid_ctx *c, const u64 *d_edges, u64 raw, u32 U, u64 *n_edges_out) {
  hipStream_t st = c->stream;
// ... 139 lines not shown
      if (join_no++ % part_world != part_rank) continue;
      if (shifted) TRY(combo_keys_sorted<WT>(c, g_word, U, cfy, kb, c->e_ky.p, c->e_vy.as<u32>()));
      const DBuf &ky = shifted ? c->e_ky : c->e_kx, &vy = shifted ? c->e_vy : c->e_vx;
      TRY(join_append(c, "edit-distance", c->e_kx.p, c->e_vx.as<u32>(), ky.p, vy.as<u32>(), U, kb <= 32, launch, raw));
    }
  }
  HIPCHK(hipGetLastError());
  if (raw == 0) return HUMID_OK;
  if (!make_unique) { *n_edges_out = raw; return HUMID_OK; }
  TRY(unique_edges(c, c->e_raw.as<u64>(), raw, U, n_edges_out));
  return HUMID_OK;
}

template <class WT>
static int paired_edges(humid_ctx *c, const WT *g_word, u32 U, u32 word_nt, u32 distance, u64 *n_edges_out) {
  hipStream_t st = c->stream;
  *n_edges_out = 0;
  if (U < 2 || distance == 0) return HUMID_OK;
  const ComboPlan plan = make_plan(word_nt, distance, U, c->force_segments);
  if (plan.ncombo == 1 && plan.key_bits == 0 && U > (1u << 18))
    return fail(c, HUMID_E_OVERFLOW, "distance %u over %u-nt words compares all pairs of %u unique words: too many neighbour pairs",
                distance, word_nt, U);
  const u32 kb = plan.key_bits ? plan.key_bits : 1;
  ENSURE(c->pd_mir, (size_t)U * sizeof(WT) + 16);
  ENSURE(c->e_kx, (size_t)U * 8);
  ENSURE(c->e_vx, (size_t)U * 4);
  ENSURE(c->e_ky, (size_t)U * 8);
  ENSURE(c->e_vy, (size_t)U * 4);
  ENSURE(c->seg_k0, (size_t)U * 8);
  ENSURE(c->seg_v0, (size_t)U * 4);
  ENSURE(c->pc, ((size_t)U + 1) * 4);
  ENSURE(c->poff, ((size_t)U + 1) * 4);
  const WT *mir = c->pd_mir.as<WT>();
  hipLaunchKernelGGL(k_pd_mirror<WT>, dim3(blocks_for(U)), dim3(256), 0, st, g_word, U, word_nt, c->pd_mir.as<WT>());
  u64 raw = 0;
  for (u32 cb = 0; cb < plan.ncombo; cb++) {
    const ComboFields cf = plan_fields(plan, cb);
    TRY(combo_keys_sorted<WT>(c, g_word, U, cf, kb, c->e_kx.p, c->e_vx.as<u32>()));
    TRY(combo_keys_sorted<WT>(c, mir, U, cf, kb, c->e_ky.p, c->e_vy.as<u32>()));
    for (u32 side = 0; side < 2; side++) {
      const WT *yw = side ? mir : g_word;
      auto launch = [&](auto fill, auto k, u64 n_pieces, u32 *pc, const u32 *poff, u64 *out) {
        constexpr bool FILL = decltype(fill)::value;
        using KT = typename decltype(k)::key_type;
        if (n_pieces)
          hipLaunchKernelGGL((k_pd_join_chunks<FILL, KT, WT>), dim3(blocks_for(n_pieces)), dim3(256), 0, st, k.kx, k.vx, k.ky, k.vy,
                             k.U, (const u32 *)c->e_runlo.as<u32>(), (const u32 *)c->e_choff.as<u32>(), (u32)n_pieces, c->walk_max,
                             g_word, yw, distance, pc, poff, out);
        else
          hipLaunchKernelGGL((k_pd_join<FILL, KT, WT>), dim3(blocks_for(k.U)), dim3(256), 0, st, k.kx, k.vx, k.ky, k.vy, k.U, g_word,
                             yw, distance, pc, poff, out, c->walk_max, &c->d_ctr[CTR_BIGMASK]);
      };
      const DBuf &ky = side ? c->e_ky : c->e_kx, &vy = side ? c->e_vy : c->e_vx;
      TRY(join_append(c, "strand-symmetric", c->e_kx.p, c->e_vx.as<u32>(), ky.p, vy.as<u32>(), U, kb <= 32, launch, raw));
    }
  }
  HIPCHK(hipGetLastError());
  if (raw == 0) return HUMID_OK;
  TRY(unique_edges(c, c->e_raw.as<u64>(), raw, U, n_edges_out));
  return HUMID_OK;
}

static int unpermute_tiled(humid_ctx *c, u32 N, bool packed, u32 *d_cid, u8 *d_keep, KernelEvent ev_mid, bool *done) {
  hipStream_t st = c->stream;
  *done = false;
  if (!c->use_tile_partition || N == 0) return HUMID_OK;
  static const u32 uw_pref = getenv("HUMID_UW_SHIFT") ? (u32)atoi(getenv("HUMID_UW_SHIFT")) : 14u;
  u32 wshift = uw_pref == 15 ? 15u : 14u;
  if (((u64)N + (1u << wshift) - 1) >> wshift > UW_MAXBINS) wshift = UW_MAXSHIFT;
  const u32 n_bins = (u32)(((u64)N + (1u << wshift) - 1) >> wshift);
  if (n_bins > UW_MAXBINS) return HUMID_OK;
  ENSURE(c->unperm_rec, ((size_t)n_bins << wshift) * 8 + (size_t)UW_MAXBINS * 4);
  u64 *rec = c->unperm_rec.as<u64>();
  u32 *ucur = (u32 *)(rec + ((size_t)n_bins << wshift));
  if (c->ucur_clean != ucur) HIPCHK(hipMemsetAsync(ucur, 0, (size_t)UW_MAXBINS * 4, st));
  c->ucur_clean = nullptr;
  const CountLeft &cl = c->count_left;
  const u32 *n_pos_dev = count_bucketed(c) ? c->pbeg.as<u32>() + cl.n_parts : (const u32 *)nullptr;
  if (count_on_records(c)) {
    const u64 mean = std::max<u64>(1, c->usable / cl.n_parts);
    const u32 chunk = (n_bins > 1024 && n_bins <= 1536) ? 7u * PT_THREADS : PT_TILE;
    const u32 B = (u32)std::min<u64>(64, std::max<u64>(1, (chunk - chunk / 8) / mean));
    const u32 grid = (cl.n_parts + B - 1) / B;
    if (n_bins <= 1024)
      hipLaunchKernelGGL(k_unperm_bins8<1024>, dim3(grid), dim3(1024), 0, st, (const u64 *)c->p8_b.as<u64>(), cl.cursor2,
                         (const u64 *)c->slot_out.as<u64>(), cl.n_parts, B, N, wshift, n_bins, ucur, rec);
    else if (n_bins <= 1536)
      hipLaunchKernelGGL((k_unperm_bins8<1536, 7>), dim3(grid), dim3(1024), 0, st, (const u64 *)c->p8_b.as<u64>(), cl.cursor2,
                         (const u64 *)c->slot_out.as<u64>(), cl.n_parts, B, N, wshift, n_bins, ucur, rec);
    else
      hipLaunchKernelGGL(k_unperm_bins8<2048>, dim3(grid), dim3(1024), 0, st, (const u64 *)c->p8_b.as<u64>(), cl.cursor2,
                         (const u64 *)c->slot_out.as<u64>(), cl.n_parts, B, N, wshift, n_bins, ucur, rec);
  }
  else
  hipLaunchKernelGGL(k_unperm_bins, dim3((N + PT_TILE - 1) / PT_TILE), dim3(1024), 0, st, c->pk_vals.as<u32>(),
                     c->pslot.as<u32>(), c->slot_out.as<u64>(), n_pos_dev, N, N, wshift, n_bins, ucur, rec);
  TRY(mark_stage(c, c->kev[ev_mid]));
  if (packed) {
    if (wshift == 14) hipLaunchKernelGGL((k_unperm_window<true, 14>), dim3(n_bins), dim3(UW_THREADS), 0, st, rec, ucur, N, d_cid, d_keep);
    else hipLaunchKernelGGL((k_unperm_window<true, 15>), dim3(n_bins), dim3(UW_THREADS), 0, st, rec, ucur, N, d_cid, d_keep);
  } else {
    if (wshift == 14) hipLaunchKernelGGL((k_unperm_window<false, 14>), dim3(n_bins), dim3(UW_THREADS), 0, st, rec, ucur, N, d_cid, d_keep);
    else hipLaunchKernelGGL((k_unperm_window<false, 15>), dim3(n_bins), dim3(UW_THREADS), 0, st, rec, ucur, N, d_cid, d_keep);
  }
  TRY(mark_kernel(c, c->kev[KEV_UNPERM_END]));
  HIPCHK(hipGetLastError());
  c->ucur_clean = ucur;
  *done = true;
  return HUMID_OK;
}

static int stage_map(humid_ctx *c, const u32 *l_cid, const u8 *l_ismax, u32 N, u32 *d_cid, u8 *d_keep) {
  hipStream_t st = c->stream;
  const u32 U = (u32)c->U;
  const bool fused = c->slots_done && l_cid == c->cid.as<u32>() && l_ismax == c->ismax.as<u8>();
  c->slots_done = false;
  if (U > 0 && !fused)
    hipLaunchKernelGGL(k_slot_results, dim3(blocks_for(U)), dim3(256), 0, st, l_cid, l_ismax,
                       c->s_first.as<u32>(), c->s_slot.as<u32>(), U, c->slot_out.as<u64>());
  TRY(mark_stage(c, c->ev[EV_CLUSTERS_DONE]));
  if (count_in_partition_order(c)) {
    bool tiled = false;
    TRY(unpermute_tiled(c, N, false, d_cid, d_keep, KEV_MAP_MID, &tiled));
    c->timing.unperm_tiled = tiled;
    if (!tiled) {
      u32 *packed = c->pk_keys.as<u32>();
      HIPCHK(hipMemsetAsync(packed, 0, (size_t)N * 4, st));
      if (count_bucketed(c))
        hipLaunchKernelGGL(k_read_map_bucket, dim3(c->count_left.n_parts), dim3(256), 0, st, c->pk_vals.as<u32>(),
                           c->pslot.as<u32>(), c->slot_out.as<u64>(), c->pbeg.as<u32>(), c->ucount.as<u32>(), N, packed);
      else
        hipLaunchKernelGGL(k_read_map_part, dim3(grid_stride_blocks(N)), dim3(256), 0, st, c->pk_vals.as<u32>(),
                           c->pslot.as<u32>(), c->slot_out.as<u64>(), N, packed);
      TRY(mark_kernel(c, c->kev[KEV_MAP_MID]));
      hipLaunchKernelGGL(k_split_out, dim3(grid_stride_blocks(N)), dim3(256), 0, st, packed, N, d_cid, d_keep);
    }
  } else
    hipLaunchKernelGGL(k_read_map, dim3(grid_stride_blocks(N)), dim3(256), 0, st, c->slot_of_read.as<u32>(),
                       c->slot_out.as<u64>(), N, d_cid, d_keep);
  TRY(mark_frame(c, c->ev[EV_PASS_END]));
  HIPCHK(hipGetLastError());
  return HUMID_OK;
}

static int gkey_check(humid_ctx *c) {
  if (c->pass_kind == RUN_PLAIN) return HUMID_OK;
  const u32 seen = *(volatile u32 *)&c->h_ctr[CTR_N + 1];
  if (seen == c->gk_epoch && c->pass_kind >= RUN_KEYED) return fail(c, HUMID_E_INVALID, "internal: a usable read's key was not ranked");
  if (seen == c->gk_epoch) return fail(c, HUMID_E_INVALID, "a usable read has a group >= n_groups");
  return HUMID_OK;
}

static int gkey_bad_word(humid_ctx *c, u32 **bad) {
  if (c->h_ctr_dev && !c->no_poll) { *bad = (u32 *)&c->h_ctr_dev[CTR_N + 1]; return HUMID_OK; }
  if (!c->gk_bad.p) {
    ENSURE(c->gk_bad, 16);
    HIPCHK(hipMemsetAsync(c->gk_bad.p, 0, 16, c->stream));
  }
  *bad = c->gk_bad.as<u32>();
  return HUMID_OK;
}
static int gkey_bad_fetch(humid_ctx *c, const u32 *bad) {
  if (bad == c->gk_bad.as<u32>()) HIPCHK(hipMemcpyAsync(&c->h_ctr[CTR_N + 1], bad, 4, hipMemcpyDeviceToHost, c->stream));
  return HUMID_OK;
}

static int check_run_args(humid_ctx *c, u64 n_reads, u32 word_nt, u32 method, u32 max_nt = 32) {
  if (word_nt == 0) return fail(c, HUMID_E_INVALID, "word_nt must be >= 1");
  if (word_nt > max_nt) return fail(c, HUMID_E_UNSUPPORTED, "word_nt %u > %u is not supported by this entry point", word_nt, max_nt);
  if (method > 1) return fail(c, HUMID_E_INVALID, "method must be 0 (directional) or 1 (maximum)");
  if (n_reads > 0x7fffffffull) return fail(c, HUMID_E_OVERFLOW, "n_reads %llu exceeds 2^31-1", (ull)n_reads);
  return HUMID_OK;
}

template <class F>
static int with_word_type(u32 word_nt, F f) { return word_nt > 32 ? f((const W2 *)nullptr) : f((const u64 *)nullptr); }

static inline const u64 *edges_or_empty(const u64 *edges, u64 n_edges) {
  static const u64 no_edges = 0;
  return n_edges ? edges : &no_edges;
}
template <class WT>
static int graph_stage(humid_ctx *c, const WT *g_word, const u32 *g_cnt, u32 U, u32 word_nt, u32 distance, u32 method, humid_summary &s,
                       u32 &n_pair_segs, bool given = false, const u64 *edges = nullptr, u64 n_edges = 0) {
  const u64 *ext = given ? edges_or_empty(edges, n_edges) : nullptr;
  if (!given) n_edges = 0;
  return c->use_compact ? stage_graph_compact<WT>(c, g_word, g_cnt, U, word_nt, distance, method, s, n_pair_segs, ext, n_edges)
                        : stage_graph<WT>(c, g_word, g_cnt, U, word_nt, distance, method, s, n_pair_segs, ext, n_edges);
}

template <class WT>
static int run_device(humid_ctx *c, const WT *d_words, const u8 *d_filt, u64 n_reads, u32 word_nt,
                      u32 distance, u32 method, u32 *d_cid, u8 *d_keep, humid_summary *sum) {
  if (!c) return HUMID_E_INVALID;
  constexpr bool WIDE = sizeof(WT) == 16;
  state_reset(c);
  TRY(check_run_args(c, n_reads, word_nt, method, 64));
  if (WIDE != (word_nt > 32)) return fail(c, HUMID_E_INVALID, "word layout does not match word_nt");
  if (WIDE && ((uintptr_t)d_words & 15)) return fail(c, HUMID_E_INVALID, "wide words must be 16-byte aligned on the device");
  if (n_reads && (!d_words || !d_filt || !d_cid || !d_keep)) return fail(c, HUMID_E_INVALID, "null buffer");
  HIPCHK(hipSetDevice(c->device));
  hipStream_t st = c->stream;
  const u32 N = (u32)n_reads;
// ... 1034 lines not shown
```

humid_amd/csrc/stage_count.hip.h:

```cpp
#pragma once

static inline void count_publish(humid_ctx *c, CountRoad road, u32 n_parts = 0, bool part_tiled = false, const u32 *cursor2 = nullptr) {
  c->count_left = CountLeft{road, n_parts, part_tiled, cursor2};
}

static int ensure_walk_order(humid_ctx *c, size_t n, size_t wsize) {
  ENSURE(c->s_word, n * wsize);
  ENSURE(c->s_slot, n * 4);
  ENSURE(c->s_cnt, n * 4);
  ENSURE(c->s_first, n * 4);
  return HUMID_OK;
}

static int stage_count_global(humid_ctx *c, const u64 *d_words, const u8 *d_filt, u32 N, u32 word_nt,
                              u64 range_lo, u64 range_hi, u64 expected_reads, humid_summary &s) {
  hipStream_t st = c->stream;
  if (expected_reads == 0 || expected_reads > N) expected_reads = N;
  u32 cap_log2 = 10;
  while (((u64)1 << cap_log2) < expected_reads + expected_reads / 2) cap_log2++;
  const u64 cap = (u64)1 << cap_log2;
  c->cap_log2 = cap_log2;
  ENSURE(c->table, (cap + 1) * sizeof(Slot));
  ENSURE(c->slot_out, (cap + 1) * 8);
  ENSURE(c->slot_of_read, (size_t)N * 4);
  ENSURE(c->uniq_slot, (size_t)expected_reads * 4 + 4);
  ENSURE(c->uniq_word, (size_t)expected_reads * 8 + 8);
  TRY(mark_frame(c, c->ev[EV_PASS_START]));
  HIPCHK(hipMemsetAsync(c->d_ctr, 0, CTR_N * sizeof(ull), st));
  HIPCHK(hipMemsetAsync(c->table.p, 0xff, (cap + 1) * sizeof(Slot), st));
  TRY(mark_frame(c, c->kev[KEV_INSERT_BEGIN]));
  hipLaunchKernelGGL(k_hash_insert, dim3(grid_stride_blocks(N)), dim3(256), 0, st, d_words, d_filt, N,
                     c->table.as<Slot>(), cap_log2, c->slot_of_read.as<u32>(), range_lo, range_hi,
                     (u32)(cap - cap / 8), c->d_ctr);
  TRY(mark_frame(c, c->kev[KEV_INSERT_END]));
  hipLaunchKernelGGL(k_compact_table, dim3(COMPACT_BLOCKS), dim3(256), 0, st,
                     c->table.as<Slot>(), (u32)(cap + 1), c->uniq_word.as<u64>(), c->uniq_slot.as<u32>(),
                     (u32)expected_reads, c->d_ctr);
  HIPCHK(hipGetLastError());
  TRY(read_counters(c));
  if (c->h_ctr[CTR_OVERFULL])
    return fail(c, HUMID_E_INVALID, "hash table over-full: more reads fell into this range than expected_reads");
  count_publish(c, COUNT_GLOBAL);
  const u32 U = (u32)c->h_ctr[CTR_UNIQUE];
  s.usable = c->usable = c->h_ctr[CTR_USABLE];
  s.unique = c->U = U;
  if (U == 0) return mark_stage(c, c->ev[EV_COUNT_END]);
  TRY(ensure_walk_order(c, U, 8));
  TRY(sort_pairs<u64, u32>(c, c->uniq_word.as<u64>(), c->s_word.as<u64>(), c->uniq_slot.as<u32>(),
                           c->s_slot.as<u32>(), U, 0, 2 * word_nt));
  hipLaunchKernelGGL(k_post_sort, dim3(blocks_for(U)), dim3(256), 0, st, c->s_slot.as<u32>(),
                     c->table.as<Slot>(), U, c->s_cnt.as<u32>(), c->s_first.as<u32>());
  TRY(mark_stage(c, c->ev[EV_COUNT_END]));
  HIPCHK(hipGetLastError());
  return HUMID_OK;
}

static inline u32 part_bits(u32 N) {
  static const u64 target = getenv("HUMID_PART_TARGET") ? (u64)std::max(32, atoi(getenv("HUMID_PART_TARGET"))) : (u64)PART_TARGET;
  u32 pb = 1;
  while (pb < 26 && (target << pb) < (u64)N) pb++;
  return pb;
}

struct KeyMap {
  u64 lo, scale;
  u32 shift;
};
static KeyMap key_map(u32 word_nt, u64 lo, u64 hi, bool within) {
  const u64 top = word_nt >= 32 ? ~0ull : (((u64)1 << (2 * word_nt)) - 1);
  if (!within) { lo = 0; hi = top; }
  if (hi > top) hi = top;
  if (lo > hi) { lo = 0; hi = top; }
  KeyMap m;
  m.lo = lo;
  const u64 span = hi - lo;
  if (span == ~0ull) { m.scale = 1; m.shift = 0; return m; }
  const u64 cnt = span + 1;
  if ((cnt & (cnt - 1)) == 0 && cnt > 1) {
    const u32 k = (u32)__builtin_ctzll(cnt);
    m.shift = 64 - k;
    m.scale = (u64)1 << m.shift;
  } else {
    m.shift = 64;
    m.scale = ~0ull / cnt;
  }
  return m;
// ... 137 lines not shown
    };
    if (ordered)
      squeeze(k_compact_padded<true>, c->s_word.as<u64>(), c->s_slot.as<u32>(), c->s_cnt.as<u32>(), c->s_first.as<u32>());
    else {
      squeeze(k_compact_padded<false>, c->uniq_word.as<u64>(), c->uniq_slot.as<u32>(), (u32 *)nullptr, (u32 *)nullptr);
      TRY(sort_pairs<u64, u32>(c, c->uniq_word.as<u64>(), c->s_word.as<u64>(), c->uniq_slot.as<u32>(),
                               c->s_slot.as<u32>(), U, 0, 2 * word_nt));
      hipLaunchKernelGGL(k_post_sort_padded, dim3(blocks_for(U)), dim3(256), 0, st, c->s_slot.as<u32>(),
                         c->pad_cf.as<uint2>(), U, c->s_cnt.as<u32>(), c->s_first.as<u32>());
    }
  }
  TRY(mark_stage(c, c->ev[EV_COUNT_END]));
  HIPCHK(hipGetLastError());
  return HUMID_OK;
}

static RecKey rec_key(const KeyMap &km) {
  RecKey rk;
  rk.lo = km.lo; rk.scale = km.scale;
  rk.pow2 = km.shift < 64 ? 1u : 0u;
  rk.z = rk.pow2 ? km.shift : 63u - (u32)__builtin_clzll(km.scale);
  rk.kbits = 64 - rk.z;
  return rk;
}

struct RecShape {
  u32 pb, d1, d2, nb1, n_parts;
  RecKey rk;
  u32 ibits, cap1;
  size_t room1, room2;
};
static bool rec_shape(const humid_ctx *c, u32 N, const KeyMap &km, bool index_in_record, RecShape *out) {
  if (!c->use_rec8 || !c->use_tile_partition || !c->pt_padded) return false;
  RecShape sh;
  sh.pb = part_bits(N);
  if (sh.pb < 6 || sh.pb > 18) return false;
  if ((((u64)N + (1u << UW_MAXSHIFT) - 1) >> UW_MAXSHIFT) > UW_MAXBINS) return false;
  sh.rk = rec_key(km);
  sh.ibits = bits_for(N);
  sh.d1 = (sh.pb + 1) / 2;
  if (sh.rk.kbits < sh.pb + 1) return false;
  if (index_in_record) {
    while (sh.d1 < 10 && sh.pb - sh.d1 > 1 && sh.rk.kbits - sh.d1 + sh.ibits > 64) sh.d1++;
    if (sh.rk.kbits - sh.d1 + sh.ibits > 64 || sh.pb - sh.d1 > 9 || sh.pb == sh.d1) return false;
  }
  sh.d2 = sh.pb - sh.d1; sh.nb1 = 1u << sh.d1; sh.n_parts = 1u << sh.pb;
  sh.cap1 = coarse_bin_room(N, sh.nb1);
  sh.room1 = (size_t)sh.nb1 * sh.cap1; sh.room2 = (size_t)sh.n_parts << P8_CAP2_LOG;
  *out = sh;
  return true;
}

struct RecWork {
  u64 *agg, *abase;
  u32 *cursor1, *cursor2, *cbase, *tprefix;
};
static int rec_work(humid_ctx *c, const RecShape &sh, size_t wsize, u64 *stamp, RecWork *out) {
  hipStream_t st = c->stream;
  ENSURE(c->p8_b, sh.room2 * 8);
  ENSURE(c->pad_word, sh.room2 * wsize);
  ENSURE(c->pad_cf, sh.room2 * 8);
  ENSURE(c->slot_out, (sh.room2 + 1) * 8);
  ENSURE(c->pbeg, (size_t)(sh.n_parts + 1) * 4);
  ENSURE(c->ucount, (size_t)(sh.n_parts + 1) * 4);
  ENSURE(c->p8_status, ((size_t)sh.n_parts + 1) * 16);
  ENSURE(c->p8_cur, ((size_t)PT_MAXBINS1 + sh.n_parts + 2 * (PT_MAXBINS1 + 1)) * 4);
  RecWork w;
  w.agg = c->p8_status.as<u64>(); w.abase = w.agg + sh.n_parts + 1;
  w.cursor1 = c->p8_cur.as<u32>(); w.cursor2 = w.cursor1 + PT_MAXBINS1;
  w.cbase = w.cursor2 + sh.n_parts; w.tprefix = w.cbase + PT_MAXBINS1 + 1;
  TRY(mark_frame(c, c->ev[EV_PASS_START]));
  ZeroList z;
  memset(&z, 0, sizeof z);
  z.p[0] = w.cursor1; z.n[0] = PT_MAXBINS1 + sh.n_parts;
  z.p[1] = (u32 *)c->d_ctr; z.n[1] = 2 * CTR_N;
  z.p[2] = (u32 *)(w.agg + sh.n_parts); z.n[2] = 2;
  hipLaunchKernelGGL(k_zero_many, dim3(32), dim3(256), 0, st, z, stamp);
  *out = w;
  return HUMID_OK;
}

template <class Squeeze>
static int rec_tail(humid_ctx *c, const RecShape &sh, const RecWork &w, u32 N, size_t wsize, u64 *stamp_k1, bool own_redo,
                    Squeeze squeeze, humid_summary &s, bool *done) {
  hipStream_t st = c->stream;
  TRY(exscan_in<u64>(c, PtrIn<u64>{w.agg}, w.abase, (u64)sh.n_parts + 1, stamp_k1));
  TRY(ensure_walk_order(c, (size_t)N + 1, wsize));
  const u32 *totals = (const u32 *)(w.abase + sh.n_parts);
  const bool early = c->overlap_waits;
  if (early) TRY(read_counters_begin(c, totals, totals + 1));
  squeeze();
  TRY(mark_stage(c, c->ev[EV_COUNT_END]));
  HIPCHK(hipGetLastError());
  if (early) TRY(read_counters_end(c, true));
  else TRY(read_counters(c, totals, totals + 1));
  const u64 special = c->h_ctr[CTR_SPECIAL], overfull = c->h_ctr[CTR_OVERFULL];
  const u32 U = (u32)(c->h_ctr[CTR_N - 1] & 0xffffffffull);
  const u64 usable = c->h_ctr[CTR_N - 2] & 0xffffffffull;
  if (getenv("HUMID_TRACE_COUNT"))
    fprintf(stderr, "[rec count%s] N %u pb %u kbits %u ibits %u cap1 %u special %llu overfull %llu unique %u usable %llu\n",
            wsize == 8 ? "" : ", wide", N, sh.pb, sh.rk.kbits, sh.ibits, sh.cap1, (ull)special, (ull)overfull, U, (ull)usable);
  if (special || overfull) {
    if (own_redo) {
      c->timing.stamp_ok = c->timing.stamp_live = c->timing.stamp_timed = false;
      if (special) { c->pt_padded = false; road_taken(c, HUMID_ROAD_PART_PADDED_REDO); }
    }
    return HUMID_OK;
  }
  count_publish(c, COUNT_REC, sh.n_parts, true, w.cursor2);
  s.usable = c->usable = usable;
  s.unique = c->U = U;
  *done = true;
  return HUMID_OK;
}

static int stage_count_rec(humid_ctx *c, const u64 *d_words, const u8 *d_filt, u32 N, u32 word_nt, u64 range_lo, u64 range_hi,
                           const KeyMap &km, humid_summary &s, bool *done) {
  hipStream_t st = c->stream;
  *done = false;
  RecShape sh;
  if (!rec_shape(c, N, km, true, &sh)) return HUMID_OK;
  const u32 pb = sh.pb, d1 = sh.d1, d2 = sh.d2, nb1 = sh.nb1, n_parts = sh.n_parts, ibits = sh.ibits, cap1 = sh.cap1;
  const RecKey &rk = sh.rk;
  ENSURE(c->p8_a, sh.room1 * 8);
  const bool stamp = c->timing.stamp_ok;
  u64 *const sp = stamp ? c->d_stamp : nullptr;
  c->timing.stamp_live = stamp;
  c->timing.stamp_timed = stamp && c->timing.lean;
  RecWork w;
  TRY(rec_work(c, sh, 8, sp ? sp + STAMP_START : (u64 *)nullptr, &w));
  const bool check_range = !(range_lo == 0 && range_hi == ~0ull);
  const Reads8 src{d_words, d_filt, range_lo, range_hi, check_range ? 1u : 0u, rk};
  const u32 tiles1 = (N + PT_TILE - 1) / PT_TILE, tiles2 = tiles1 + nb1;
  hipLaunchKernelGGL((k_p8_scatter1<Reads8, 1024>), dim3(tiles1), dim3(1024), 0, st, src, N, rk.kbits, d1, ibits, cap1, w.cursor1,
                     c->p8_a.as<u64>(), c->d_ctr);
  if (c->static_tiles) {
    TRY(mark_kernel(c, c->kev[KEV_PART_BEGIN]));
    hipLaunchKernelGGL(k_p8_scatter2<true>, dim3(nb1 * ((cap1 + PT_TILE - 1) / PT_TILE)), dim3(1024), 0, st, (const u64 *)c->p8_a.as<u64>(),
                       (const u32 *)w.cursor1, (const u32 *)nullptr, rk.kbits, d1, d2, ibits, cap1, w.cursor2, c->p8_b.as<u64>(), c->d_ctr);
  } else {
    hipLaunchKernelGGL(k_pt_scan1, dim3(1), dim3(1024), 0, st, (const u32 *)w.cursor1, d1, d2, w.cbase, w.tprefix, c->pbeg.as<u32>(),
                       c->ucount.as<u32>() + n_parts, cap1);
    TRY(mark_kernel(c, c->kev[KEV_PART_BEGIN]));
    hipLaunchKernelGGL(k_p8_scatter2<false>, dim3(tiles2), dim3(1024), 0, st, (const u64 *)c->p8_a.as<u64>(), (const u32 *)w.tprefix,
                       (const u32 *)w.cbase, rk.kbits, d1, d2, ibits, cap1, w.cursor2, c->p8_b.as<u64>(), c->d_ctr);
  }
  TRY(mark_kernel(c, c->kev[KEV_PART_END]));
  TRY(mark_frame(c, c->kev[KEV_INSERT_BEGIN]));
  hipLaunchKernelGGL(k_dedup_rec, dim3(n_parts), dim3(256), 0, st, c->p8_b.as<u64>(), (const u32 *)w.cursor2, N, pb, d1, ibits, rk,
                     c->pad_word.as<u64>(), c->pad_cf.as<uint2>(), w.agg, c->d_ctr, sp ? sp + STAMP_K0 : (u64 *)nullptr);
  TRY(mark_frame(c, c->kev[KEV_INSERT_END]));
  auto squeeze = [&] {
    hipLaunchKernelGGL(k_compact_padded8, dim3(blocks_for((u64)n_parts * 64)), dim3(256), 0, st, c->pad_word.as<u64>(),
                       c->pad_cf.as<uint2>(), (const u64 *)w.agg, (const u64 *)w.abase, n_parts, c->s_word.as<u64>(),
                       c->s_slot.as<u32>(), c->s_cnt.as<u32>(), c->s_first.as<u32>());
  };
  return rec_tail(c, sh, w, N, 8, sp ? sp + STAMP_K1 : (u64 *)nullptr, true, squeeze, s, done);
}

static int stage_count_rec_wide(humid_ctx *c, const W2 *d_words, const u8 *d_filt, u32 N, u32 word_nt, const KeyMap &km,
                                humid_summary &s, bool *done) {
  hipStream_t st = c->stream;
  *done = false;
  RecShape sh;
  if (!rec_shape(c, N, km, false, &sh)) return HUMID_OK;
  const u32 pb = sh.pb, d1 = sh.d1, d2 = sh.d2, nb1 = sh.nb1, n_parts = sh.n_parts, cap1 = sh.cap1;
  const RecKey &rk = sh.rk;
  const u32 hbits = 2 * (word_nt - 32);
  ENSURE(c->pw_a, sh.room1 * 16);
  ENSURE(c->pw_ai, sh.room1 * 4);
  ENSURE(c->pw_b, sh.room2 * 16);
  ENSURE(c->pw_bi, sh.room2 * 4);
  RecWork w;
  TRY(rec_work(c, sh, sizeof(W2), nullptr, &w));
  const u32 tiles1 = (N + PT_TILE - 1) / PT_TILE, tiles2 = tiles1 + nb1;
  hipLaunchKernelGGL(k_pw_scatter<1>, dim3(tiles1), dim3(1024), 0, st, d_words, d_filt, (const u32 *)nullptr, N, hbits, rk,
                     (const u32 *)nullptr, (const u32 *)nullptr, d1, d2, cap1, w.cursor1, c->pw_a.as<W2>(), c->pw_ai.as<u32>(), c->d_ctr);
  hipLaunchKernelGGL(k_pt_scan1, dim3(1), dim3(1024), 0, st, (const u32 *)w.cursor1, d1, d2, w.cbase, w.tprefix, c->pbeg.as<u32>(),
                     c->ucount.as<u32>() + n_parts, cap1);
  TRY(mark_kernel(c, c->kev[KEV_PART_BEGIN]));
  hipLaunchKernelGGL(k_pw_scatter<2>, dim3(tiles2), dim3(1024), 0, st, (const W2 *)c->pw_a.as<W2>(), (const u8 *)nullptr,
                     (const u32 *)c->pw_ai.as<u32>(), N, hbits, rk, (const u32 *)w.tprefix, (const u32 *)w.cbase, d1, d2, cap1, w.cursor2,
                     c->pw_b.as<W2>(), c->pw_bi.as<u32>(), c->d_ctr);
  TRY(mark_kernel(c, c->kev[KEV_PART_END]));
  TRY(mark_frame(c, c->kev[KEV_INSERT_BEGIN]));
  auto count = [&](auto kernel) {
    hipLaunchKernelGGL(kernel, dim3(n_parts), dim3(256), 0, st, (const W2 *)c->pw_b.as<W2>(), (const u32 *)c->pw_bi.as<u32>(),
                       (const u32 *)w.cursor2, hbits, rk, N, pb, c->pad_word.as<W2>(), c->pad_cf.as<uint2>(), w.agg, c->p8_b.as<u64>(),
                       c->d_ctr);
  };
  count(k_dedup_wide_rec<9, 512, 0, WL_SMALL_LEN>);
  if (N > WL_SMALL_LEN) count(k_dedup_wide_rec<10, 1024, WL_SMALL_LEN, WL_STAGE>);
  TRY(mark_frame(c, c->kev[KEV_INSERT_END]));
  auto squeeze = [&] {
    hipLaunchKernelGGL(k_compact_padded8_wide, dim3(blocks_for((u64)n_parts * 64)), dim3(256), 0, st, (const W2 *)c->pad_word.as<W2>(),
                       (const uint2 *)c->pad_cf.as<uint2>(), (const u64 *)w.agg, (const u64 *)w.abase, n_parts, c->s_word.as<W2>(),
                       c->s_slot.as<u32>(), c->s_cnt.as<u32>(), c->s_first.as<u32>());
  };
  return rec_tail(c, sh, w, N, sizeof(W2), nullptr, false, squeeze, s, done);
}

static inline bool memo_matches(const OrderedMemo &m, u32 N, u32 word_nt, const KeyMap &km) {
  return m.valid && m.n == N && m.nt == word_nt && m.lo == km.lo && m.scale == km.scale;
}
static inline void memo_set(OrderedMemo &m, u32 N, u32 word_nt, const KeyMap &km, bool fits) {
  m = OrderedMemo{true, fits, N, word_nt, km.lo, km.scale};
}

static int prefix_fits_ordered(humid_ctx *c, const u64 *d_words, const u8 *d_filt, u32 N, u32 word_nt,
                               const KeyMap &km, bool *fits) {
  *fits = false;
  if (memo_matches(c->ordered_memo, N, word_nt, km)) {
    *fits = c->ordered_memo.fits;
    return HUMID_OK;
  }
  const u32 bits = 2 * word_nt < 12 ? 2 * word_nt : 12;
  const u32 n_bins = 1u << bits;
  if (N < 65536) return HUMID_OK;
  const u32 n_sample = N < (1u << 19) ? N : (1u << 19);
  ENSURE(c->small, (size_t)n_bins * 4);
  HIPCHK(hipMemsetAsync(c->small.p, 0, (size_t)n_bins * 4, c->stream));
  hipLaunchKernelGGL(k_top_hist, dim3(128), dim3(1024), n_bins * 4, c->stream, d_words, d_filt, n_sample,
                     km.lo, km.scale, bits, c->small.as<u32>());
  std::vector<u32> h(n_bins);
  HIPCHK(hipMemcpyAsync(h.data(), c->small.p, (size_t)n_bins * 4, hipMemcpyDeviceToHost, c->stream));
  HIPCHK(hipGetLastError());
  HIPCHK(hipStreamSynchronize(c->stream));
  const u32 pb = part_bits(N);
  double worst = 0;
  if (pb >= bits) {
    u32 mx = 0;
    for (u32 v : h) if (v > mx) mx = v;
    worst = (double)mx / (double)(1u << (pb - bits));
  } else {
    const u32 per = 1u << (bits - pb);
    for (u32 b = 0; b < n_bins; b += per) {
      u64 t = 0;
      for (u32 k = 0; k < per; k++) t += h[b + k];
      if ((double)t > worst) worst = (double)t;
    }
  }
  worst *= (double)N / (double)n_sample;
  *fits = worst * 1.5 <= (double)LDS_FILL_LIMIT;
  memo_set(c->ordered_memo, N, word_nt, km, *fits);
  return HUMID_OK;
}

static int stage_count(humid_ctx *c, const u64 *d_words, const u8 *d_filt, u32 N, u32 word_nt,
                       u64 range_lo, u64 range_hi, u64 expected_reads, humid_summary &s, bool within = false) {
  const bool full_range = (range_lo == 0 && range_hi == ~0ull);
  if (c->count_mode == 0 && (full_range || within)) {
    const KeyMap km = key_map(word_nt, range_lo, range_hi, within);
    bool overflowed = false;
    bool ordered = c->count_order == 1;
    if (c->count_order < 0) TRY(prefix_fits_ordered(c, d_words, d_filt, N, word_nt, km, &ordered));
    if (ordered) {
      bool done = false;
      TRY(stage_count_rec(c, d_words, d_filt, N, word_nt, range_lo, range_hi, km, s, &done));
      if (done) return HUMID_OK;
      TRY(stage_count_lds(c, d_words, d_filt, N, word_nt, range_lo, range_hi, km, true, s, &overflowed));
      if (!overflowed) return HUMID_OK;
      memo_set(c->ordered_memo, N, word_nt, km, false);
    }
    TRY(stage_count_lds(c, d_words, d_filt, N, word_nt, range_lo, range_hi, km, false, s, &overflowed));
    if (!overflowed) return HUMID_OK;
  }
  return stage_count_global(c, d_words, d_filt, N, word_nt, range_lo, range_hi, expected_reads, s);
}

static int sorted_count_front(humid_ctx *c, u32 N, size_t word_bytes) {
  hipStream_t st = c->stream;
  ENSURE(c->pk_keys, (size_t)N * 8);
  ENSURE(c->pad_word, (size_t)N * 8);
  ENSURE(c->pk_vals, (size_t)N * 4);
  ENSURE(c->uniq_slot, (size_t)N * 4 + 4);
  ENSURE(c->pslot, (size_t)N * 4);
  ENSURE(c->w_sorted, (size_t)N * word_bytes);
  ENSURE(c->w_head, ((size_t)N + 1) * 4);
  ENSURE(c->w_hpos, ((size_t)N + 1) * 4);
  TRY(mark_frame(c, c->ev[EV_PASS_START]));
  HIPCHK(hipMemsetAsync(c->d_ctr, 0, CTR_N * sizeof(ull), st));
  TRY(mark_frame(c, c->kev[KEV_INSERT_BEGIN]));
// ... 111 lines not shown
```

Before: 19.57 billion reads/s.

## Emit dense per-unique results and encode first-read flag in partition records

The dedup record kernel now packs each unique's local index into the record and flags whether that read is the family's first occurrence. Finalization writes a dense per-unique result array with the cluster id and max bit, four leaves per thread with a vectorized store. The unpermute kernel then reads that dense array by partition base plus local index, instead of gathering 64-bit slot_out entries and comparing read ids. This swaps a random 8-byte gather for a denser 4-byte lookup, at the cost of extra state flags that must be kept valid across stages and more kernel template variants.

Measured after the change: 19.83 billion reads/s (median of 6 runs). 1.01x the previous value.

```diff
diff --git a/humid_amd/csrc/humid_exchange.hip b/humid_amd/csrc/humid_exchange.hip
--- a/humid_amd/csrc/humid_exchange.hip
+++ b/humid_amd/csrc/humid_exchange.hip
@@ -360,6 +360,7 @@
                          (u32)u_local, 0u, c->x_lcid.as<u32>(), c->x_lismax.as<u8>(), c->xo_ldeg.as<u32>(),
                          (const u32 *)c->s_first.as<u32>(), (const u32 *)c->s_slot.as<u32>(), c->slot_out.as<u64>(), true);
       c->slots_done = true;
+      c->results_dense = false;
       l_cid = c->x_lcid.as<u32>();
       l_ismax = c->x_lismax.as<u8>();
     }
@@ -790,6 +791,7 @@
                        (u32)u_local, (u32)creators_before, c->x_lcid.as<u32>(), c->x_lismax.as<u8>(), c->xo_ldeg.as<u32>(),
                        (const u32 *)c->s_first.as<u32>(), (const u32 *)c->s_slot.as<u32>(), c->slot_out.as<u64>());
     c->slots_done = true;
+    c->results_dense = false;
     HIPCHK(hipGetLastError());
     l_cid = c->x_lcid.as<u32>();
     l_ismax = c->x_lismax.as<u8>();
@@ -980,10 +982,12 @@
   *n_packed = N;
   if (N == 0) return HUMID_OK;
   if (U && (!d_local_cluster_id || !d_local_is_max)) return fail(c, HUMID_E_INVALID, "null buffer");
+  if (!c->slots_done) c->results_dense = false;
   if (U > 0 && !c->slots_done)
     hipLaunchKernelGGL(k_slot_results, dim3(blocks_for(U)), dim3(256), 0, st, d_local_cluster_id, d_local_is_max,
                        c->s_first.as<u32>(), c->s_slot.as<u32>(), U, c->slot_out.as<u64>());
   c->slots_done = false;
+  struct Spent { humid_ctx *c; ~Spent() { c->results_dense = false; } } spent{c};
   ENSURE(c->own_packed, ((size_t)N + 1) * 4);
   TRY(mark_kernel(c, c->kev[KEV_DENSE_MAP_BEGIN]));
   bool tiled = false;
@@ -1717,6 +1721,7 @@
   for (u32 q = 0; q <= n_shards; q++)
     if (shard_begin[q] > N || (q && shard_begin[q] < shard_begin[q - 1])) return fail(c, HUMID_E_INVALID, "shard_begin must ascend within [0, n_reads]");
   if (U && (!d_local_cluster_id || !d_local_is_max)) return fail(c, HUMID_E_INVALID, "null buffer");
+  c->results_dense = false;
   if (U > 0)
     hipLaunchKernelGGL(k_slot_results, dim3(blocks_for(U)), dim3(256), 0, st, d_local_cluster_id, d_local_is_max,
                        c->s_first.as<u32>(), c->s_slot.as<u32>(), U, c->slot_out.as<u64>());
diff --git a/humid_amd/csrc/humid_hip.hip b/humid_amd/csrc/humid_hip.hip
--- a/humid_amd/csrc/humid_hip.hip
+++ b/humid_amd/csrc/humid_hip.hip
@@ -199,6 +199,10 @@
   }
   if (strcmp(key, "static_tiles") == 0) {
     c->static_tiles = value != 0;
+    return HUMID_OK;
+  }
+  if (strcmp(key, "dense_results") == 0) {
+    c->dense_results = value != 0;
     return HUMID_OK;
   }
   if (strcmp(key, "padded_partition") == 0) {
diff --git a/humid_amd/csrc/kernels_cgraph.hip.h b/humid_amd/csrc/kernels_cgraph.hip.h
--- a/humid_amd/csrc/kernels_cgraph.hip.h
+++ b/humid_amd/csrc/kernels_cgraph.hip.h
@@ -594,6 +594,50 @@
   if (cid_out) { cid_out[u] = id; ismax_out[u] = mx ? 1 : 0; }
 }
 
+#define FL_GROUP 4u
+static __global__ void __launch_bounds__(256)
+k_finalize_leaves_dense(BitRank in_graph, BitRank noncreator, const u32 *__restrict__ nodes, const u32 *__restrict__ cl_of,
+                        const u32 *__restrict__ maxleaf, u32 n, u32 *__restrict__ res,
+                        const u32 *__restrict__ any_pair = nullptr, const u32 *__restrict__ pair_res = nullptr) {
+  HUMID_GUARD_LAST_VGPR();
+  const u32 u0 = (blockIdx.x * blockDim.x + threadIdx.x) * FL_GROUP;
+  if (u0 >= n) return;
+  const u32 sh = u0 & 31;
+  const u32 paired = (pair_res ? any_pair : in_graph.bits)[u0 >> 5] >> sh;
+  const u32 nc = noncreator.bits[u0 >> 5] >> sh;
+  const u32 r0 = br_rank(noncreator, u0);
+  u32 out[FL_GROUP];
+#pragma unroll
+  for (u32 k = 0; k < FL_GROUP; k++) {
+    const u32 u = u0 + k;
+    out[k] = 0;
+    if (u >= n) continue;
+    if (!((paired >> k) & 1u)) {
+      out[k] = (1u + u - (r0 + (u32)__popc(nc & ((1u << k) - 1u)))) | 0x80000000u;
+      continue;
+    }
+    u32 g = u;
+    bool mx = true;
+    if (br_test(in_graph, u)) {
+      const u32 c = br_rank(in_graph, u);
+      const u32 cc = cl_of[c] - 1u;
+      g = nodes[cc];
+      mx = maxleaf[cc] == c;
+    } else if (pair_res) {
+      const u32 p = pair_res[u];
+      g = p & 0x7fffffffu;
+      mx = (p >> 31) != 0;
+    }
+    out[k] = (1u + g - br_rank(noncreator, g)) | (mx ? 0x80000000u : 0u);
+  }
+  if (u0 + FL_GROUP <= n) *(uint4 *)(res + u0) = make_uint4(out[0], out[1], out[2], out[3]);
+  else {
+#pragma unroll
+    for (u32 k = 0; k < FL_GROUP; k++)
+      if (u0 + k < n) res[u0 + k] = out[k];
+  }
+}
+
 static __global__ void __launch_bounds__(256)
 k_expand_leaves(BitRank in_graph, const u32 *__restrict__ nodes, const u32 *__restrict__ cdeg, const u32 *__restrict__ ccl_of,
                 const u32 *__restrict__ cmaxleaf, const u64 *__restrict__ ccl_size, const u32 *__restrict__ cnt, u32 n,
diff --git a/humid_amd/csrc/kernels_part8.hip.h b/humid_amd/csrc/kernels_part8.hip.h
--- a/humid_amd/csrc/kernels_part8.hip.h
+++ b/humid_amd/csrc/kernels_part8.hip.h
@@ -214,6 +214,9 @@
 }
 #define DR_WORDS (DR_SLOTS / 32u)
 #define DR_EARLY 1u
+#define P8_FIRST 0x80000000u
+#define P8_SLOT(hi) ((hi) & ~P8_FIRST)
+template <bool FIRST>
 static __global__ void __launch_bounds__(256)
 k_dedup_rec(u64 *recs, const u32 *__restrict__ cursor2, u32 n_reads, u32 pb, u32 d1, u32 ibits, RecKey rk,
             u64 *__restrict__ pad_word, uint2 *__restrict__ pad_cf, u64 *__restrict__ agg, ull *ctr, u64 *stamp = nullptr) {
@@ -309,7 +312,8 @@
     const uint2 cf = lcf[sl];
     pad_word[beg + r] = rk.word(k);
     pad_cf[beg + r] = cf;
-    lcf[sl].y = r;
+    if (FIRST) lcf[sl].x = cf.x | (r << 16);
+    else lcf[sl].y = r;
   }
   if (threadIdx.x == 0) agg[g] = ((u64)n << 32) | n_uniq;
   PH(4);
@@ -319,8 +323,15 @@
   for (u32 q = 0; q < P8_RPT; q++) {
     const u32 i = threadIdx.x + 256u * q;
     if (i >= n) continue;
-    const u32 li = sq[q] != NONE32 ? lcf[sq[q]].y : NONE32;
-    recs[beg + i] = ((u64)(li < n ? (u32)beg + li : NOSLOT) << 32) | (u32)(rq[q] & imask);
+    const u32 v = (u32)(rq[q] & imask);
+    if (FIRST) {
+      const uint2 e = sq[q] != NONE32 ? lcf[sq[q]] : make_uint2(NONE32, NONE32);
+      const u32 li = e.x >> 16;
+      recs[beg + i] = ((u64)(li < n ? ((u32)beg + li) | (e.y == v ? P8_FIRST : 0u) : NOSLOT) << 32) | v;
+    } else {
+      const u32 li = sq[q] != NONE32 ? lcf[sq[q]].y : NONE32;
+      recs[beg + i] = ((u64)(li < n ? (u32)beg + li : NOSLOT) << 32) | v;
+    }
   }
   PH(6);
   PH_END(0, 6, (g & 255u) == 77u);
@@ -344,15 +355,19 @@
   }
 }
 
-template <u32 NBMAX, u32 UIPT = 8u>
+enum : u32 { UB_PLAIN = 0, UB_MASKED = 1, UB_DENSE = 2 };
+template <u32 NBMAX, u32 UIPT = 8u, u32 FORM = UB_PLAIN>
 __global__ void __launch_bounds__(1024, NBMAX <= 1536 ? 8 : 4)
-k_unperm_bins8(const u64 *__restrict__ recs, const u32 *__restrict__ cursor2, const u64 *__restrict__ slot_out, u32 n_parts,
+k_unperm_bins8(const u64 *__restrict__ recs, const u32 *__restrict__ cursor2, const u64 *__restrict__ slot_out,
+               const u32 *__restrict__ res, const u64 *__restrict__ abase, u32 n_unique, u32 n_parts,
                u32 B, u32 n_reads, u32 wshift, u32 n_bins, u32 *ucur, u64 *__restrict__ rec) {
   HUMID_GUARD_LAST_VGPR();
+  constexpr bool DENSE = FORM == UB_DENSE;
   constexpr u32 UTILE = PT_THREADS * UIPT;
   __shared__ u64 srec[UTILE];
   __shared__ u32 cnt[NBMAX], loff[NBMAX + 1], goff[NBMAX], wsum[16];
   __shared__ u32 bpre[65];
+  __shared__ u32 ub[DENSE ? 64 : 1];
   PH_DECL;
   PH(0);
   const u32 g0 = blockIdx.x * B;
@@ -360,6 +375,7 @@
   const u32 nbk = (n_parts - g0 < B) ? n_parts - g0 : B;
   if (threadIdx.x < 64) {
     u32 c = threadIdx.x < nbk ? cursor2[g0 + threadIdx.x] : 0u;
+    if (DENSE) ub[threadIdx.x] = threadIdx.x < nbk ? (u32)abase[g0 + threadIdx.x] : 0u;
     if (c > P8_CAP2) c = P8_CAP2;
     u32 incl = c;
     incl = wave_incl_scan(incl);
@@ -385,18 +401,25 @@
         while (bpre[lo] > r) lo--;
         while (bpre[lo + 1] <= r) lo++;
         in[q] = recs[((size_t)(g0 + lo) << P8_CAP2_LOG) + (r - bpre[lo])];
-        binrank[q] = 0;
+        binrank[q] = DENSE ? ub[lo] : 0u;
       }
     }
     PH(2);
 #pragma unroll
     for (u32 q = 0; q < UIPT; q++) {
       if (binrank[q] == NONE32) continue;
-      const u32 r = (u32)in[q], sl = (u32)(in[q] >> 32);
+      const u32 r = (u32)in[q], hi = (u32)(in[q] >> 32);
+      const u32 u = binrank[q] + (hi & (P8_CAP2 - 1u));
       binrank[q] = NONE32;
-      if (r < n_reads && sl != NOSLOT) {
-        const u64 o = slot_out[sl];
-        const u32 c = (u32)o | (((u32)(o >> 32) == r) ? 0x80000000u : 0u);
+      if (r < n_reads && hi != NOSLOT && (!DENSE || u < n_unique)) {
+        u32 c;
+        if (DENSE) {
+          const u32 o = res[u];
+          c = (o & 0x7fffffffu) | (o & hi & P8_FIRST);
+        } else {
+          const u64 o = slot_out[FORM == UB_MASKED ? P8_SLOT(hi) : hi];
+          c = (u32)o | (((u32)(o >> 32) == r) ? 0x80000000u : 0u);
+        }
         r64[q] = ((u64)c << 32) | r;
         const u32 bin = r >> wshift;
         binrank[q] = bin << 16 | atomicAdd(&cnt[bin], 1u);
diff --git a/humid_amd/csrc/pass_timing.hip.h b/humid_amd/csrc/pass_timing.hip.h
--- a/humid_amd/csrc/pass_timing.hip.h
+++ b/humid_amd/csrc/pass_timing.hip.h
@@ -38,6 +38,7 @@
   c->N = n_reads; c->U = c->E = c->M = c->C = c->usable = 0;
   c->word_nt = word_nt;
   c->gU = 0;
+  c->results_dense = false;
 }
 static inline void pass_begin(humid_ctx *c, u64 n_reads, u32 word_nt, u32 distance, u32 method) {
   pass_begin(c, n_reads, word_nt);
diff --git a/humid_amd/csrc/pipeline.hip.h b/humid_amd/csrc/pipeline.hip.h
--- a/humid_amd/csrc/pipeline.hip.h
+++ b/humid_amd/csrc/pipeline.hip.h
@@ -108,6 +108,7 @@
   u32 n_parts = 0;
   bool part_tiled = false;
   const u32 *cursor2 = nullptr;
+  const u64 *abase = nullptr;
 };
 struct OrderedMemo {
   bool valid = false, fits = false;
@@ -237,6 +238,9 @@
   OrderedMemo ordered_memo;
   u32 g_wpr = 1;
   bool slots_done = false;
+  bool dense_results = true;
+  bool results_dense = false;
+  DBuf res_u;
   int count_mode = 0;
   u32 force_segments = 0;
   bool force_comm = false;
@@ -352,6 +356,7 @@
 static inline bool count_bucketed(const humid_ctx *c) { return c->count_left.n_parts != 0; }
 static inline bool count_on_records(const humid_ctx *c) { return c->count_left.road == COUNT_REC; }
 static inline bool count_part_timed(const humid_ctx *c) { return c->count_left.part_tiled; }
+static inline bool count_flags_first(const humid_ctx *c) { return count_on_records(c) && c->count_left.abase != nullptr; }
 static inline u32 count_mode_used(const humid_ctx *c) {
   static const u32 mode[] = {1u, 0u, 2u, 2u | 0x100u, 3u};
   return mode[c->count_left.road];
@@ -1126,6 +1131,7 @@
                      own ? c->s_slot.as<u32>() : (const u32 *)nullptr,
                      own ? c->slot_out.as<u64>() : (u64 *)nullptr);
   c->slots_done = own;
+  c->results_dense = false;
   HIPCHK(hipGetLastError());
   n_pair_segs_out = n_pair_segs;
   return HUMID_OK;
@@ -1498,15 +1504,22 @@
   const GraphArrays g = cg_arrays(c);
   const bool own = ((const void *)g_word == c->s_word.p) && U == (u32)c->U;
   if (!own) { ENSURE(c->cid, (size_t)U * 4); ENSURE(c->ismax, (size_t)U); }
-  hipLaunchKernelGGL(k_finalize_leaves, dim3(blocks_for(U)), dim3(256), 0, st,
-                     BitRank{split ? c->cg_rbits.as<u32>() : c->cg_bits.as<u32>(), c->cg_blk.as<u32>()},
-                     BitRank{c->cg_nbits.as<u32>(), c->cg_nblk.as<u32>()}, c->cg_nodes.as<u32>(), (const u32 *)g.cl_of,
-                     (const u32 *)g.maxleaf, U, own ? c->s_first.as<u32>() : (const u32 *)nullptr,
-                     own ? c->s_slot.as<u32>() : (const u32 *)nullptr, own ? c->slot_out.as<u64>() : (u64 *)nullptr,
-                     own ? (u32 *)nullptr : c->cid.as<u32>(), own ? (u8 *)nullptr : c->ismax.as<u8>(),
-                     split ? (const u32 *)c->cg_bits.as<u32>() : (const u32 *)nullptr,
-                     split ? (const u32 *)c->cg_pres.as<u32>() : (const u32 *)nullptr);
+  const bool dense = own && count_flags_first(c);
+  const BitRank in_graph{split ? c->cg_rbits.as<u32>() : c->cg_bits.as<u32>(), c->cg_blk.as<u32>()};
+  const BitRank noncreator{c->cg_nbits.as<u32>(), c->cg_nblk.as<u32>()};
+  const u32 *any_pair = split ? (const u32 *)c->cg_bits.as<u32>() : (const u32 *)nullptr;
+  const u32 *pair_res = split ? (const u32 *)c->cg_pres.as<u32>() : (const u32 *)nullptr;
+  if (dense) {
+    ENSURE(c->res_u, ((size_t)U + 1) * 4);
+    hipLaunchKernelGGL(k_finalize_leaves_dense, dim3(blocks_for(U, 256 * FL_GROUP)), dim3(256), 0, st, in_graph, noncreator,
+                       c->cg_nodes.as<u32>(), (const u32 *)g.cl_of, (const u32 *)g.maxleaf, U, c->res_u.as<u32>(), any_pair, pair_res);
+  } else
+    hipLaunchKernelGGL(k_finalize_leaves, dim3(blocks_for(U)), dim3(256), 0, st, in_graph, noncreator, c->cg_nodes.as<u32>(),
+                       (const u32 *)g.cl_of, (const u32 *)g.maxleaf, U, own ? c->s_first.as<u32>() : (const u32 *)nullptr,
+                       own ? c->s_slot.as<u32>() : (const u32 *)nullptr, own ? c->slot_out.as<u64>() : (u64 *)nullptr,
+                       own ? (u32 *)nullptr : c->cid.as<u32>(), own ? (u8 *)nullptr : c->ismax.as<u8>(), any_pair, pair_res);
   c->slots_done = own;
+  c->results_dense = dense;
   c->cg_valid = true;
   HIPCHK(hipGetLastError());
   n_pair_segs_out = nseg < 8 ? nseg : 8;
@@ -1812,15 +1825,18 @@
     const u32 chunk = (n_bins > 1024 && n_bins <= 1536) ? 7u * PT_THREADS : PT_TILE;
     const u32 B = (u32)std::min<u64>(64, std::max<u64>(1, (chunk - chunk / 8) / mean));
     const u32 grid = (cl.n_parts + B - 1) / B;
-    if (n_bins <= 1024)
-      hipLaunchKernelGGL(k_unperm_bins8<1024>, dim3(grid), dim3(1024), 0, st, (const u64 *)c->p8_b.as<u64>(), cl.cursor2,
-                         (const u64 *)c->slot_out.as<u64>(), cl.n_parts, B, N, wshift, n_bins, ucur, rec);
-    else if (n_bins <= 1536)
-      hipLaunchKernelGGL((k_unperm_bins8<1536, 7>), dim3(grid), dim3(1024), 0, st, (const u64 *)c->p8_b.as<u64>(), cl.cursor2,
-                         (const u64 *)c->slot_out.as<u64>(), cl.n_parts, B, N, wshift, n_bins, ucur, rec);
-    else
-      hipLaunchKernelGGL(k_unperm_bins8<2048>, dim3(grid), dim3(1024), 0, st, (const u64 *)c->p8_b.as<u64>(), cl.cursor2,
-                         (const u64 *)c->slot_out.as<u64>(), cl.n_parts, B, N, wshift, n_bins, ucur, rec);
+    const bool dense = c->results_dense && count_flags_first(c);
+    auto bins8 = [&](auto kernel) {
+      hipLaunchKernelGGL(kernel, dim3(grid), dim3(1024), 0, st, (const u64 *)c->p8_b.as<u64>(), cl.cursor2,
+                         (const u64 *)c->slot_out.as<u64>(), (const u32 *)c->res_u.as<u32>(), cl.abase, (u32)c->U, cl.n_parts, B, N,
+                         wshift, n_bins, ucur, rec);
+    };
+    auto form = [&](auto plain, auto masked, auto dense_form) {
+      if (dense) bins8(dense_form); else if (count_flags_first(c)) bins8(masked); else bins8(plain);
+    };
+    if (n_bins <= 1024) form(k_unperm_bins8<1024>, k_unperm_bins8<1024, 8, UB_MASKED>, k_unperm_bins8<1024, 8, UB_DENSE>);
+    else if (n_bins <= 1536) form(k_unperm_bins8<1536, 7>, k_unperm_bins8<1536, 7, UB_MASKED>, k_unperm_bins8<1536, 7, UB_DENSE>);
+    else form(k_unperm_bins8<2048>, k_unperm_bins8<2048, 8, UB_MASKED>, k_unperm_bins8<2048, 8, UB_DENSE>);
   }
   else
   hipLaunchKernelGGL(k_unperm_bins, dim3((N + PT_TILE - 1) / PT_TILE), dim3(1024), 0, st, c->pk_vals.as<u32>(),
@@ -1845,10 +1861,12 @@
   const u32 U = (u32)c->U;
   const bool fused = c->slots_done && l_cid == c->cid.as<u32>() && l_ismax == c->ismax.as<u8>();
   c->slots_done = false;
+  if (!fused) c->results_dense = false;
   if (U > 0 && !fused)
     hipLaunchKernelGGL(k_slot_results, dim3(blocks_for(U)), dim3(256), 0, st, l_cid, l_ismax,
                        c->s_first.as<u32>(), c->s_slot.as<u32>(), U, c->slot_out.as<u64>());
   TRY(mark_stage(c, c->ev[EV_CLUSTERS_DONE]));
+  struct Spent { humid_ctx *c; ~Spent() { c->results_dense = false; } } spent{c};
   if (count_in_partition_order(c)) {
     bool tiled = false;
     TRY(unpermute_tiled(c, N, false, d_cid, d_keep, KEV_MAP_MID, &tiled));
diff --git a/humid_amd/csrc/stage_count.hip.h b/humid_amd/csrc/stage_count.hip.h
--- a/humid_amd/csrc/stage_count.hip.h
+++ b/humid_amd/csrc/stage_count.hip.h
@@ -1,7 +1,9 @@
 #pragma once
 
-static inline void count_publish(humid_ctx *c, CountRoad road, u32 n_parts = 0, bool part_tiled = false, const u32 *cursor2 = nullptr) {
-  c->count_left = CountLeft{road, n_parts, part_tiled, cursor2};
+static inline void count_publish(humid_ctx *c, CountRoad road, u32 n_parts = 0, bool part_tiled = false, const u32 *cursor2 = nullptr,
+                                 const u64 *abase = nullptr) {
+  c->count_left = CountLeft{road, n_parts, part_tiled, cursor2, abase};
+  c->results_dense = false;
 }
 
 static int ensure_walk_order(humid_ctx *c, size_t n, size_t wsize) {
@@ -305,7 +307,7 @@
 
 template <class Squeeze>
 static int rec_tail(humid_ctx *c, const RecShape &sh, const RecWork &w, u32 N, size_t wsize, u64 *stamp_k1, bool own_redo,
-                    Squeeze squeeze, humid_summary &s, bool *done) {
+                    bool first_bit, Squeeze squeeze, humid_summary &s, bool *done) {
   hipStream_t st = c->stream;
   TRY(exscan_in<u64>(c, PtrIn<u64>{w.agg}, w.abase, (u64)sh.n_parts + 1, stamp_k1));
   TRY(ensure_walk_order(c, (size_t)N + 1, wsize));
@@ -330,7 +332,7 @@
     }
     return HUMID_OK;
   }
-  count_publish(c, COUNT_REC, sh.n_parts, true, w.cursor2);
+  count_publish(c, COUNT_REC, sh.n_parts, true, w.cursor2, first_bit ? (const u64 *)w.abase : (const u64 *)nullptr);
   s.usable = c->usable = usable;
   s.unique = c->U = U;
   *done = true;
@@ -370,15 +372,19 @@
   }
   TRY(mark_kernel(c, c->kev[KEV_PART_END]));
   TRY(mark_frame(c, c->kev[KEV_INSERT_BEGIN]));
-  hipLaunchKernelGGL(k_dedup_rec, dim3(n_parts), dim3(256), 0, st, c->p8_b.as<u64>(), (const u32 *)w.cursor2, N, pb, d1, ibits, rk,
-                     c->pad_word.as<u64>(), c->pad_cf.as<uint2>(), w.agg, c->d_ctr, sp ? sp + STAMP_K0 : (u64 *)nullptr);
+  const bool first_bit = c->dense_results;
+  auto count = [&](auto kernel) {
+    hipLaunchKernelGGL(kernel, dim3(n_parts), dim3(256), 0, st, c->p8_b.as<u64>(), (const u32 *)w.cursor2, N, pb, d1, ibits, rk,
+                       c->pad_word.as<u64>(), c->pad_cf.as<uint2>(), w.agg, c->d_ctr, sp ? sp + STAMP_K0 : (u64 *)nullptr);
+  };
+  if (first_bit) count(k_dedup_rec<true>); else count(k_dedup_rec<false>);
   TRY(mark_frame(c, c->kev[KEV_INSERT_END]));
   auto squeeze = [&] {
     hipLaunchKernelGGL(k_compact_padded8, dim3(blocks_for((u64)n_parts * 64)), dim3(256), 0, st, c->pad_word.as<u64>(),
                        c->pad_cf.as<uint2>(), (const u64 *)w.agg, (const u64 *)w.abase, n_parts, c->s_word.as<u64>(),
                        c->s_slot.as<u32>(), c->s_cnt.as<u32>(), c->s_first.as<u32>());
   };
-  return rec_tail(c, sh, w, N, 8, sp ? sp + STAMP_K1 : (u64 *)nullptr, true, squeeze, s, done);
+  return rec_tail(c, sh, w, N, 8, sp ? sp + STAMP_K1 : (u64 *)nullptr, true, first_bit, squeeze, s, done);
 }
 
 static int stage_count_rec_wide(humid_ctx *c, const W2 *d_words, const u8 *d_filt, u32 N, u32 word_nt, const KeyMap &km,
@@ -420,7 +426,7 @@
                        (const uint2 *)c->pad_cf.as<uint2>(), (const u64 *)w.agg, (const u64 *)w.abase, n_parts, c->s_word.as<W2>(),
                        c->s_slot.as<u32>(), c->s_cnt.as<u32>(), c->s_first.as<u32>());
   };
-  return rec_tail(c, sh, w, N, sizeof(W2), nullptr, false, squeeze, s, done);
+  return rec_tail(c, sh, w, N, sizeof(W2), nullptr, false, false, squeeze, s, done);
 }
 
 static inline bool memo_matches(const OrderedMemo &m, u32 N, u32 word_nt, const KeyMap &km) {
```
